# eth-ait/GaussianHaircut

Hardware: NVIDIA H100
Metric: fwd+bwd Gaussians/s at 500k G, 1080p (higher is better)
Workload: dtype f32

## Files before the change

### gaussianhaircut_b200/_C.py

```python
from __future__ import annotations

import ctypes as C
from typing import Optional, Tuple

import torch

from . import _capi
from ._alloc import empty_rows, row_capacity

NUM_CHANNELS = 10

_GRAD_LAYOUT = (("rotations", 4), ("colors", NUM_CHANNELS), ("opacity", 1), ("means3D", 3), ("scales", 3),
                ("means2D", 3), ("conic", 4), ("cov3D", 6))
_N_TRAINABLE_SEGMENTS = 5
GRAD_FLOATS_TRAINABLE_NATIVE = 4 + NUM_CHANNELS + 1 + 3 + 3
GRAD_FLOATS_PER_GAUSSIAN = sum(n for _, n in _GRAD_LAYOUT)


def _seg_floats(P: int, n: int) -> int:
    return (P * n + 3) // 4 * 4


def arena_floats(P: int) -> int:
    return sum(_seg_floats(P, n) for _, n in _GRAD_LAYOUT)


def trainable_floats(P: int) -> int:
    return sum(_seg_floats(P, n) for _, n in _GRAD_LAYOUT[:_N_TRAINABLE_SEGMENTS])


def _ptr(t: Optional[torch.Tensor]):
    if t is None or t.numel() == 0:
        return None
    return C.c_void_p(t.data_ptr())


def _prep(t: torch.Tensor, name: str, device: torch.device, align: int = 4) -> torch.Tensor:
    if t.numel() == 0:
        return t
    if t.dtype != torch.float32:
        raise RuntimeError(f"expected scalar type Float but found {t.dtype} for argument '{name}'")
    if t.device != device:
        raise RuntimeError(f"argument '{name}' is on {t.device}, expected {device}")
    t = t.contiguous()
    if t.data_ptr() % align:
        t = t.clone()
    return t


def _stream(device: torch.device):
    return C.c_void_p(torch.cuda.current_stream(device).cuda_stream)


def rasterize_gaussians(
    background: torch.Tensor, means3D: torch.Tensor, means2D_precomp: torch.Tensor,
    colors: torch.Tensor, opacity: torch.Tensor, scales: torch.Tensor, rotations: torch.Tensor,
    scale_modifier: float, cov3D_precomp: torch.Tensor, conic_precomp: torch.Tensor,
    viewmatrix: torch.Tensor, projmatrix: torch.Tensor, tan_fovx: float, tan_fovy: float,
    image_height: int, image_width: int, sh: torch.Tensor, degree: int, campos: torch.Tensor,
    prefiltered: bool, debug: bool,
) -> Tuple[int, torch.Tensor, torch.Tensor, torch.Tensor, torch.Tensor, torch.Tensor]:
    if means3D.ndim != 2 or means3D.size(1) != 3:
        raise RuntimeError("means3D must have dimensions (num_points, 3)")
    lib = _capi.load()
    device = means3D.device
    if device.type != "cuda":
        raise RuntimeError("gaussianhaircut_b200 rasterizer: tensors must live on a CUDA device (no CPU path)")
    P, H, W = int(means3D.size(0)), int(image_height), int(image_width)
    byte_opts = dict(dtype=torch.uint8, device=device)

    if P == 0:
        return (0, torch.zeros((NUM_CHANNELS, H, W), dtype=torch.float32, device=device),
                torch.zeros((0,), dtype=torch.int32, device=device),
                torch.empty(0, **byte_opts), torch.empty(0, **byte_opts), torch.empty(0, **byte_opts))

    with torch.cuda.device(device):
        means3D = _prep(means3D, "means3D", device)
        colors = _prep(colors, "colors", device, align=8)
        opacity = _prep(opacity, "opacity", device)
        scales = _prep(scales, "scales", device)
        rotations = _prep(rotations, "rotations", device, align=16)
        cov3D_precomp = _prep(cov3D_precomp, "cov3D_precomp", device)
        conic_precomp = _prep(conic_precomp, "conic_precomp", device)
        viewmatrix = _prep(viewmatrix, "viewmatrix", device)
        projmatrix = _prep(projmatrix, "projmatrix", device)
        background = _prep(background, "background", device)
        M = int(sh.size(1)) if sh.numel() != 0 else 0

        geom_bytes, img_bytes, geom_cap = C.c_size_t(), C.c_size_t(), C.c_size_t()
        _capi.check(lib.gh_forward_workspace_sizes(P, W, H, C.byref(geom_bytes), C.byref(img_bytes)))
        _capi.check(lib.gh_forward_workspace_sizes(row_capacity(P), W, H, C.byref(geom_cap), None))
        geomBuffer = torch.empty(geom_cap.value, **byte_opts)[:geom_bytes.value]
        imgBuffer = torch.empty(img_bytes.value, **byte_opts)
        radii = empty_rows(P, (), torch.int32, device)
        out_color = torch.empty((NUM_CHANNELS, H, W), dtype=torch.float32, device=device)
        stream = _stream(device)

        n_rendered, max_len = C.c_int(0), C.c_int(0)
        _capi.check(lib.gh_forward_preprocess(
            P, int(degree), M, W, H,
            _ptr(means3D), _ptr(means2D_precomp), _ptr(sh), _ptr(colors), _ptr(opacity),
            _ptr(scales), float(scale_modifier), _ptr(rotations),
            _ptr(cov3D_precomp), _ptr(conic_precomp),
            _ptr(viewmatrix), _ptr(projmatrix), _ptr(campos),
            float(tan_fovx), float(tan_fovy), int(bool(prefiltered)),
            _ptr(radii), _ptr(geomBuffer), _ptr(imgBuffer),
            C.byref(n_rendered), C.byref(max_len), int(bool(debug)), stream))
        R = int(n_rendered.value)

        bin_bytes = C.c_size_t()
        _capi.check(lib.gh_binning_workspace_size(R, C.byref(bin_bytes)))
        binningBuffer = torch.empty(bin_bytes.value, **byte_opts)
        _capi.check(lib.gh_forward_render(
            P, W, H, _ptr(background), _ptr(colors), _ptr(radii),
            _ptr(geomBuffer), _ptr(binningBuffer), _ptr(imgBuffer),
            R, int(max_len.value), _ptr(out_color), int(bool(debug)), stream))
    return R, out_color, radii, geomBuffer, binningBuffer, imgBuffer


def alloc_forward_workspaces(P: int, W: int, H: int, device: torch.device):
    lib = _capi.load()
    byte_opts = dict(dtype=torch.uint8, device=device)
    geom_bytes, img_bytes, geom_cap = C.c_size_t(), C.c_size_t(), C.c_size_t()
    _capi.check(lib.gh_forward_workspace_sizes(P, W, H, C.byref(geom_bytes), C.byref(img_bytes)))
    _capi.check(lib.gh_forward_workspace_sizes(row_capacity(P), W, H, C.byref(geom_cap), None))
    geomBuffer = torch.empty(geom_cap.value, **byte_opts)[:geom_bytes.value]
    imgBuffer = torch.empty(img_bytes.value, **byte_opts)
    radii = empty_rows(P, (), torch.int32, device)
    return geomBuffer, imgBuffer, radii


def forward_render(background: torch.Tensor, colors: torch.Tensor, radii: torch.Tensor, geomBuffer: torch.Tensor,
                   imgBuffer: torch.Tensor, num_rendered: int, max_tile_len: int, image_height: int, image_width: int,
                   debug: bool = False):
    lib = _capi.load()
    device = colors.device
    P, H, W = int(colors.shape[0]), int(image_height), int(image_width)
    with torch.cuda.device(device):
        background = _prep(background, "background", device)
        colors = _prep(colors, "colors", device, align=8)
        out_color = torch.empty((NUM_CHANNELS, H, W), dtype=torch.float32, device=device)
        bin_bytes = C.c_size_t()
        _capi.check(lib.gh_binning_workspace_size(int(num_rendered), C.byref(bin_bytes)))
        binningBuffer = torch.empty(bin_bytes.value, dtype=torch.uint8, device=device)
        _capi.check(lib.gh_forward_render(
            P, W, H, _ptr(background), _ptr(colors), _ptr(radii),
            _ptr(geomBuffer), _ptr(binningBuffer), _ptr(imgBuffer),
            int(num_rendered), int(max_tile_len), _ptr(out_color), int(bool(debug)), _stream(device)))
    return out_color, binningBuffer


def alloc_grad_arena(P: int, device: torch.device, zero: bool = True, storage: torch.Tensor | None = None):
    n = arena_floats(P)
    if storage is not None:
        if storage.dtype != torch.float32 or storage.numel() < n or not storage.is_contiguous():
            raise RuntimeError("gradient arena storage must be a contiguous float32 tensor of at least _C.arena_floats(P) elements")
        flat = storage.view(-1)[:n]
        if zero:
            flat.zero_()
    else:
        alloc = torch.zeros if zero else torch.empty
        flat = alloc(n, dtype=torch.float32, device=device)
    views, off = {}, 0
    for name, k in _GRAD_LAYOUT:
        views[name] = flat[off:off + P * k].view(P, k)
        off += _seg_floats(P, k)
    return flat, views


def rasterize_gaussians_backward_arena(
    background, means3D, radii, colors, scales, rotations, scale_modifier, cov3D_precomp, conic_precomp,
    viewmatrix, projmatrix, tan_fovx, tan_fovy, dL_dout_color, sh, degree, campos,
    geomBuffer, R, binningBuffer, imageBuffer, debug, arena_storage=None,
):
    lib = _capi.load()
    device = means3D.device
    P = int(means3D.size(0))
    H, W = int(dL_dout_color.size(1)), int(dL_dout_color.size(2))
    M = int(sh.size(1)) if sh.numel() != 0 else 0
    flat, g = alloc_grad_arena(P, device, zero=False, storage=arena_storage)
    dL_dsh = torch.zeros((P, M, 3), dtype=torch.float32, device=device)
    if P != 0:
        with torch.cuda.device(device):
            means3D = _prep(means3D, "means3D", device)
            colors = _prep(colors, "colors", device, align=8)
            scales = _prep(scales, "scales", device)
            rotations = _prep(rotations, "rotations", device, align=16)
            cov3D_precomp = _prep(cov3D_precomp, "cov3D_precomp", device)
            conic_precomp = _prep(conic_precomp, "conic_precomp", device)
            viewmatrix = _prep(viewmatrix, "viewmatrix", device)
            projmatrix = _prep(projmatrix, "projmatrix", device)
            background = _prep(background, "background", device)
            dL_dout_color = _prep(dL_dout_color, "dL_dout_color", device)
            radii = radii.contiguous()
            _capi.check(lib.gh_backward(
                P, int(degree), M, int(R), W, H,
                _ptr(background), _ptr(means3D), _ptr(sh), _ptr(colors),
                _ptr(scales), float(scale_modifier), _ptr(rotations),
                _ptr(cov3D_precomp), _ptr(conic_precomp),
                _ptr(viewmatrix), _ptr(projmatrix), _ptr(campos),
                float(tan_fovx), float(tan_fovy), _ptr(radii),
                _ptr(geomBuffer), _ptr(binningBuffer), _ptr(imageBuffer),
                _ptr(dL_dout_color),
                _ptr(g["means2D"]), _ptr(g["conic"]), _ptr(g["opacity"]), _ptr(g["colors"]),
                _ptr(g["means3D"]), _ptr(g["cov3D"]), _ptr(dL_dsh), _ptr(g["scales"]), _ptr(g["rotations"]),
                int(bool(debug)), _stream(device)))
    return flat, g, dL_dsh


def rasterize_gaussians_backward_records(background, means3D, radii, colors, conic_precomp, viewmatrix, projmatrix,
                                         tan_fovx, tan_fovy, dL_dout_color, campos, geomBuffer, R, binningBuffer,
                                         imageBuffer, debug) -> None:
    lib = _capi.load()
    device = means3D.device
    P = int(means3D.size(0))
    if P == 0:
        return
    H, W = int(dL_dout_color.size(1)), int(dL_dout_color.size(2))
    if conic_precomp is None or conic_precomp.numel() == 0:
        raise RuntimeError("rasterize_gaussians_backward_records needs the conic_precomp call shape")
    with torch.cuda.device(device):
        dL = _prep(dL_dout_color, "dL_dout_color", device)
        _capi.check(lib.gh_backward(
            P, 0, 0, int(R), W, H,
            _ptr(background), _ptr(means3D), None, _ptr(colors),
            None, 1.0, None, None, _ptr(conic_precomp),
            _ptr(viewmatrix), _ptr(projmatrix), _ptr(campos),
            float(tan_fovx), float(tan_fovy), _ptr(radii),
            _ptr(geomBuffer), _ptr(binningBuffer), _ptr(imageBuffer),
            _ptr(dL),
            None, None, None, None, None, None, None, None, None,
            int(bool(debug)), _stream(device)))


def rasterize_gaussians_backward(
    background: torch.Tensor, means3D: torch.Tensor, radii: torch.Tensor, colors: torch.Tensor,
    scales: torch.Tensor, rotations: torch.Tensor, scale_modifier: float,
    cov3D_precomp: torch.Tensor, conic_precomp: torch.Tensor,
    viewmatrix: torch.Tensor, projmatrix: torch.Tensor, tan_fovx: float, tan_fovy: float,
    dL_dout_color: torch.Tensor, sh: torch.Tensor, degree: int, campos: torch.Tensor,
    geomBuffer: torch.Tensor, R: int, binningBuffer: torch.Tensor, imageBuffer: torch.Tensor,
    debug: bool,
):
    _flat, g, dL_dsh = rasterize_gaussians_backward_arena(
        background, means3D, radii, colors, scales, rotations, scale_modifier, cov3D_precomp, conic_precomp,
        viewmatrix, projmatrix, tan_fovx, tan_fovy, dL_dout_color, sh, degree, campos,
        geomBuffer, R, binningBuffer, imageBuffer, debug)
    P = int(means3D.size(0))
    return (g["means2D"], g["colors"], g["opacity"], g["means3D"], g["cov3D"],
            g["conic"].view(P, 2, 2), dL_dsh, g["scales"], g["rotations"])


def mark_visible(means3D: torch.Tensor, viewmatrix: torch.Tensor, projmatrix: torch.Tensor) -> torch.Tensor:
    lib = _capi.load()
    device = means3D.device
    P = int(means3D.size(0))
    present = torch.zeros((P,), dtype=torch.bool, device=device)
    if P != 0:
        with torch.cuda.device(device):
            means3D = _prep(means3D, "means3D", device)
            viewmatrix = _prep(viewmatrix, "viewmatrix", device)
            projmatrix = _prep(projmatrix, "projmatrix", device)
            _capi.check(lib.gh_mark_visible(P, _ptr(means3D), _ptr(viewmatrix), _ptr(projmatrix),
                                            _ptr(present), _stream(device)))
    return present


def debug_export(P: int, W: int, H: int, R: int, geomBuffer, binningBuffer, imgBuffer):
    lib = _capi.load()
    device = geomBuffer.device
    T = ((W + 15) // 16) * ((H + 15) // 16)
    out = {
        "keys": torch.zeros(R, dtype=torch.int64, device=device),
        "point_list": torch.zeros(R, dtype=torch.int32, device=device),
        "ranges": torch.zeros((T, 2), dtype=torch.int32, device=device),
        "final_T": torch.zeros(H * W, dtype=torch.float32, device=device),
        "n_contrib": torch.zeros(H * W, dtype=torch.int32, device=device),
        "depths": torch.zeros(P, dtype=torch.float32, device=device),
        "means2D": torch.zeros((P, 2), dtype=torch.float32, device=device),
        "conic_opacity": torch.zeros((P, 4), dtype=torch.float32, device=device),
    }
    with torch.cuda.device(device):
        _capi.check(lib.gh_debug_export(
            P, W, H, R, _ptr(geomBuffer), _ptr(binningBuffer), _ptr(imgBuffer),
            _ptr(out["keys"]), _ptr(out["point_list"]), _ptr(out["ranges"]),
            _ptr(out["final_T"]), _ptr(out["n_contrib"]),
            _ptr(out["depths"]), _ptr(out["means2D"]), _ptr(out["conic_opacity"]), _stream(device)))
    return out
```

### gaussianhaircut_b200/_capi.py

```python
from __future__ import annotations

import ctypes as C
import os

_HERE = os.path.dirname(os.path.abspath(__file__))
LIB_PATH = os.path.join(_HERE, "lib", "libgh_raster.so")

GH_OK = 0
GH_E_INVALID_ARG = 1
GH_E_NO_COLORS = 2
GH_E_CUDA = 3
GH_E_PREFILTERED = 4

ABI_VERSION = 3

_p = C.c_void_p
_i = C.c_int
_f = C.c_float
_ll = C.c_longlong
_sz = C.c_size_t

SIGNATURES = {
    "gh_abi_version": (_i, []),
    "gh_num_channels": (_i, []),
    "gh_last_error": (C.c_char_p, []),
    "gh_kernel_launch_count": (C.c_ulonglong, []),
    "gh_stage_timing_enable": (None, [_i]),
    "gh_stage_timing_read": (_i, [C.POINTER(C.c_double), C.POINTER(C.c_ulonglong), _i]),
    "gh_forward_workspace_sizes": (_i, [_i, _i, _i, C.POINTER(_sz), C.POINTER(_sz)]),
    "gh_binning_workspace_size": (_i, [_ll, C.POINTER(_sz)]),
    "gh_forward_preprocess": (_i, [
        _i, _i, _i, _i, _i,
        _p, _p, _p, _p, _p,
        _p, _f, _p,
        _p, _p,
        _p, _p, _p,
        _f, _f, _i,
        _p,
        _p, _p,
        C.POINTER(_i), C.POINTER(_i),
        _i, _p]),
    "gh_forward_render": (_i, [
        _i, _i, _i, _p, _p, _p, _p, _p, _p, _i, _i, _p, _i, _p]),
    "gh_backward": (_i, [
        _i, _i, _i, _i, _i, _i,
        _p,
        _p, _p, _p,
        _p, _f, _p,
        _p, _p,
        _p, _p, _p,
        _f, _f,
        _p,
        _p, _p, _p,
        _p,
        _p, _p, _p, _p,
        _p, _p, _p, _p, _p,
        _i, _p]),
    "gh_mark_visible": (_i, [_i, _p, _p, _p, _p, _p]),
    "gh_adam_step": (_i, [_i, _p, _p, _p, _p, _p, _p, _f, _f, _f, _i, _p, _p, _p, _p]),
    "gh_image_loss_workspace_size": (_i, [_i, _i, C.POINTER(C.c_size_t)]),
    "gh_allreduce_p2p": (_i, [_p, _p, C.c_ulonglong, _i, _i, C.c_size_t, C.c_size_t, C.c_uint, _p, _p, _p]),
    "gh_image_loss": (_i, [_i, _i, _p, _p, _p, _p, _p, _f, _f, _f, _f, _p, _p, _p, _p]),
    "gh_project_workspace_size": (_i, [_i, C.POINTER(C.c_size_t)]),
    "gh_project_forward": (_i, [
        _i, _i, _i,
        _p, _p, _p, _p,
        _p, _p,
        _p, _p, _p,
        _p, _p, _p,
        _f, _f, _f, _i, C.c_uint, _f,
        _p, _p, _p, _p, _p, _p,
        _p]),
    "gh_project_forward_binned": (_i, [
        _i, _i, _i,
        _p, _p, _p, _p,
        _p, _p,
        _p, _p, _p,
        _p, _p, _p,
        _f, _f, _f, _i, C.c_uint, _f,
        _p, _p, _p, _p, _p, _p,
        _p, _p, _p, C.POINTER(C.c_int), C.POINTER(C.c_int),
        _p]),
    "gh_project_backward": (_i, [
        _i, _i, _i,
        _p, _p, _p, _p,
        _p, _p,
        _p, _p, _p,
        _p, _p, _p,
        _f, _f, _f, _i, C.c_uint, _f,
        _p,
        _p,
        _p, _p, _p, _p,
        _p, _p, _p, _p, _p, _p,
        _p, _p, _p, _p, _p,
        _p, _p, _p]),
    "gh_densify_classify": (_i, [_i, _p, _p, _p, _p, _f, _f, _f, _f, _p, _p]),
    "gh_densify_scatter": (_i, [_i, _i, _p, _p, _p, _p, _p, _p, _p, _i, _i, _i, _p, _p, _i, _i, _i, _p, _i, _p]),
    "gh_debug_export": (_i, [_i, _i, _i, _ll, _p, _p, _p, _p, _p, _p, _p, _p, _p, _p, _p, _p]),
}

_lib = None


class GhError(RuntimeError):

    def __init__(self, code: int, message: str):
        super().__init__(message)
        self.code = code


def load() -> C.CDLL:
    global _lib
    if _lib is not None:
        return _lib
    if not os.path.isfile(LIB_PATH):
        raise RuntimeError(
            f"gaussianhaircut_b200: native library not found at {LIB_PATH}. "
            "Build it with `python -m gaussianhaircut_b200.build` (needs nvcc; there is no CPU fallback).")
    lib = C.CDLL(LIB_PATH)
    for name, (res, args) in SIGNATURES.items():
        fn = getattr(lib, name)
        fn.restype = res
        fn.argtypes = args
    if lib.gh_abi_version() != ABI_VERSION:
        raise RuntimeError(f"libgh_raster.so ABI {lib.gh_abi_version()} != binding ABI {ABI_VERSION}; rebuild")
    _lib = lib
    return lib


STAGE_NAMES = ("preprocess", "tile_scan", "emit", "tile_sort", "blend_forward", "blend_backward",
               "preprocess_backward")


def stage_timing_read():
    lib = load()
    n = len(STAGE_NAMES)
    ms = (C.c_double * n)()
    calls = (C.c_ulonglong * n)()
    lib.gh_stage_timing_read(ms, calls, n)
    return {STAGE_NAMES[i]: (ms[i], int(calls[i])) for i in range(n)}


def check(status: int) -> None:
    if status != GH_OK:
        msg = load().gh_last_error().decode("utf-8", "replace")
        raise GhError(status, msg or f"libgh_raster error {status}")
```

### gaussianhaircut_b200/csrc/gh_api.cu

```cuda
#include "gh_common.cuh"
#include "gh_kernels.h"
#include "../../include/gh_rasterizer.h"

#include <atomic>
#include <cstdio>
#include <cstring>
#include <mutex>

static thread_local char g_err[512] = "";
void gh_clear_error() { g_err[0] = 0; }
int gh_set_error(int code, const char* msg) {
    std::snprintf(g_err, sizeof(g_err), "%s", msg ? msg : "");
    return code;
}

namespace {

int gh_fail(int code, const char* msg) { return gh_set_error(code, msg); }

int gh_check_cuda(cudaError_t e, const char* what) {
    if (e == cudaSuccess) return GH_OK;
    std::snprintf(g_err, sizeof(g_err), "[CUDA ERROR] %s: %s", what, cudaGetErrorString(e));
    return GH_E_CUDA;
}

#define GH_STAGE(stream, debug, what)                                             \
    do {                                                                           \
        cudaError_t e__ = cudaGetLastError();                                      \
        if (e__ == cudaSuccess && (debug)) e__ = cudaStreamSynchronize(stream);    \
        if (e__ != cudaSuccess) return gh_check_cuda(e__, what);                   \
    } while (0)

enum { GH_ST_PREPROCESS = 0, GH_ST_TILE_SCAN, GH_ST_EMIT, GH_ST_TILE_SORT, GH_ST_BLEND_FWD, GH_ST_BLEND_BWD,
       GH_ST_PREPROCESS_BWD, GH_ST_COUNT };
std::atomic<bool> g_timing{false};
std::mutex g_timing_mu;
double g_stage_ms[GH_ST_COUNT] = {0};
unsigned long long g_stage_calls[GH_ST_COUNT] = {0};
std::atomic<unsigned long long> g_launches{0};

struct GhStageTimer {
    int stage; cudaStream_t stream; unsigned long long l0; bool on;
    cudaEvent_t ev0 = nullptr, ev1 = nullptr;
    GhStageTimer(int st, cudaStream_t s) : stage(st), stream(s), l0(g_launches.load()), on(g_timing.load()) {
        if (on) {
            on = (cudaEventCreate(&ev0) == cudaSuccess) && (cudaEventCreate(&ev1) == cudaSuccess);
            if (on) cudaEventRecord(ev0, stream);
        }
    }
    ~GhStageTimer() {
        if (on && g_launches.load() != l0) {
            cudaEventRecord(ev1, stream);
            cudaEventSynchronize(ev1);
            float ms = 0.f;
            if (cudaEventElapsedTime(&ms, ev0, ev1) == cudaSuccess) {
                std::lock_guard<std::mutex> lk(g_timing_mu);
                g_stage_ms[stage] += ms; g_stage_calls[stage] += 1;
            }
        }
        if (ev0) cudaEventDestroy(ev0);
        if (ev1) cudaEventDestroy(ev1);
    }
};

inline void gh_grid(int W, int H, int& gx, int& gy) {
    gx = (W + GH_BLOCK_X - 1) / GH_BLOCK_X;
    gy = (H + GH_BLOCK_Y - 1) / GH_BLOCK_Y;
}

__global__ void gh_export_keys_kernel(const uint2* __restrict__ ranges, const uint64_t* __restrict__ inst,
                                      unsigned long long* __restrict__ keys, unsigned int* __restrict__ plist)
{
    const uint2 rg = ranges[blockIdx.x];
    for (uint32_t i = rg.x + threadIdx.x; i < rg.y; i += blockDim.x) {
        const uint64_t r = inst[i];
        if (keys) keys[i] = ((unsigned long long)blockIdx.x << 32) | (r >> 32);
        if (plist) plist[i] = (unsigned int)r;
    }
}

__global__ void gh_export_geom_kernel(int P, const GhGeo* __restrict__ geo, float* __restrict__ means2D,
                                      float* __restrict__ conic_opacity)
{
    const int i = blockIdx.x * blockDim.x + threadIdx.x;
    if (i >= P) return;
    const GhGeo g = geo[i];
    if (means2D) { means2D[2 * i] = g.x; means2D[2 * i + 1] = g.y; }
    if (conic_opacity) {
        conic_opacity[4 * i + 0] = g.ca; conic_opacity[4 * i + 1] = g.cb;
        conic_opacity[4 * i + 2] = g.cc; conic_opacity[4 * i + 3] = g.op;
    }
}

}

void gh_count_launches(int n) { g_launches.fetch_add((unsigned long long)n); }

extern "C" {

int gh_abi_version(void) { return 3; }

unsigned long long gh_kernel_launch_count(void) { return g_launches.load(); }

void gh_stage_timing_enable(int on) {
    std::lock_guard<std::mutex> lk(g_timing_mu);
    g_timing.store(on != 0);
    for (int i = 0; i < GH_ST_COUNT; i++) { g_stage_ms[i] = 0.0; g_stage_calls[i] = 0; }
}

int gh_stage_timing_read(double* ms_sum, unsigned long long* calls, int capacity) {
    std::lock_guard<std::mutex> lk(g_timing_mu);
    const int n = capacity < GH_ST_COUNT ? capacity : GH_ST_COUNT;
    for (int i = 0; i < n; i++) { if (ms_sum) ms_sum[i] = g_stage_ms[i]; if (calls) calls[i] = g_stage_calls[i]; }
    return GH_ST_COUNT;
}
int gh_num_channels(void) { return GH_NUM_CHANNELS; }
const char* gh_last_error(void) { return g_err; }

int gh_forward_workspace_sizes(int P, int width, int height, size_t* geom_bytes, size_t* img_bytes)
{
    if (P < 0 || width <= 0 || height <= 0) return gh_fail(GH_E_INVALID_ARG, "gh_forward_workspace_sizes: bad P/width/height");
    int gx, gy; gh_grid(width, height, gx, gy);
    if (geom_bytes) *geom_bytes = GhGeomWS::bytes((size_t)P);
    if (img_bytes) *img_bytes = GhImgWS::bytes((size_t)width * height, (size_t)gx * gy);
    return GH_OK;
}

int gh_binning_workspace_size(long long R, size_t* binning_bytes)
{
    if (R < 0) return gh_fail(GH_E_INVALID_ARG, "gh_binning_workspace_size: negative R");
    if (binning_bytes) *binning_bytes = GhBinWS::bytes((size_t)R);
    return GH_OK;
}

int gh_forward_preprocess(
    int P, int D, int M, int width, int height,
    const float* means3D, const float* means2D_precomp, const float* shs,
    const float* colors_precomp, const float* opacities,
    const float* scales, float scale_modifier, const float* rotations,
    const float* cov3D_precomp, const float* conic_precomp,
    const float* viewmatrix, const float* projmatrix, const float* cam_pos,
    float tan_fovx, float tan_fovy, int prefiltered,
    int* radii, char* geom_buffer, char* img_buffer,
    int* num_rendered, int* max_tile_len, int debug, gh_stream_t stream_)
{
    (void)D; (void)M; (void)means2D_precomp; (void)shs; (void)cam_pos;
    cudaStream_t stream = (cudaStream_t)stream_;
    g_err[0] = 0;
    if (P <= 0 || width <= 0 || height <= 0) return gh_fail(GH_E_INVALID_ARG, "gh_forward_preprocess: P, width, height must be positive");
    if (colors_precomp == nullptr)
        return gh_fail(GH_E_NO_COLORS, "For non-RGB, provide precomputed Gaussian colors!");
    if (!means3D || !opacities || !viewmatrix || !projmatrix || !radii || !geom_buffer || !img_buffer || !num_rendered)
        return gh_fail(GH_E_INVALID_ARG, "gh_forward_preprocess: missing mandatory pointer");
    if (conic_precomp == nullptr && cov3D_precomp == nullptr && (scales == nullptr || rotations == nullptr))
        return gh_fail(GH_E_INVALID_ARG, "Please provide exactly one of either scale/rotation pair or precomputed 3D covariance!");
    if (rotations && ((size_t)rotations & 15)) return gh_fail(GH_E_INVALID_ARG, "rotations must be 16-byte aligned");
    if (((size_t)colors_precomp & 7)) return gh_fail(GH_E_INVALID_ARG, "colors_precomp must be 8-byte aligned");

    int gx, gy; gh_grid(width, height, gx, gy);
    const int T = gx * gy;
    if ((unsigned long long)gx * gx * gy >= (1ull << 32))
        return gh_fail(GH_E_INVALID_ARG, "gh_forward_preprocess: image too large (tile grid gx * gx * gy must stay below 2^32)");
    GhGeomWS geom = GhGeomWS::carve(geom_buffer, (size_t)P);
    GhImgWS img = GhImgWS::carve(img_buffer, (size_t)width * height, (size_t)T);

    cudaError_t e = cudaMemsetAsync(img.ctrl, 0, 256 + gh_align_up((size_t)T * 4, 256), stream);
    if (e != cudaSuccess) return gh_check_cuda(e, "memset(tile histogram)");

    {
        GhStageTimer t(GH_ST_PREPROCESS, stream);
        gh_launch_preprocess(P, means3D, scales, scale_modifier, rotations, opacities, cov3D_precomp,
                             conic_precomp, viewmatrix, projmatrix, width, height, tan_fovx, tan_fovy,
                             radii, geom, img, prefiltered, stream);
        g_launches += 1;
    }
    GH_STAGE(stream, debug, "preprocess");
    {
        GhStageTimer t(GH_ST_TILE_SCAN, stream);
        gh_launch_tile_scan(T, img, stream);
        g_launches += 1;
    }
    GH_STAGE(stream, debug, "tile scan");
    GhCtrl h;
    e = cudaMemcpyAsync(&h, img.ctrl, sizeof(GhCtrl), cudaMemcpyDeviceToHost, stream);
    if (e == cudaSuccess) e = cudaStreamSynchronize(stream);
    if (e != cudaSuccess) return gh_check_cuda(e, "read back num_rendered");
    *num_rendered = (int)h.num_rendered;
    if (max_tile_len) *max_tile_len = (int)h.max_tile_len;
    if (h.err_flags & GH_ERR_PREFILTERED)
        return gh_fail(GH_E_PREFILTERED, "Point is filtered although prefiltered is set. This shouldn't happen!");
    return GH_OK;
}

int gh_forward_render(
    int P, int width, int height,
    const float* background, const float* colors_precomp, const int* radii,
    char* geom_buffer, char* binning_buffer, char* img_buffer,
    int num_rendered, int max_tile_len, float* out_color, int debug, gh_stream_t stream_)
{
    cudaStream_t stream = (cudaStream_t)stream_;
    g_err[0] = 0;
    if (P <= 0 || width <= 0 || height <= 0 || num_rendered < 0) return gh_fail(GH_E_INVALID_ARG, "gh_forward_render: bad sizes");
    if (!background || !colors_precomp || !radii || !geom_buffer || !img_buffer || !out_color || (num_rendered > 0 && !binning_buffer))
        return gh_fail(GH_E_INVALID_ARG, "gh_forward_render: missing mandatory pointer");
    int gx, gy; gh_grid(width, height, gx, gy);
    const int T = gx * gy;
    GhGeomWS geom = GhGeomWS::carve(geom_buffer, (size_t)P);
    GhImgWS img = GhImgWS::carve(img_buffer, (size_t)width * height, (size_t)T);
    GhBinWS bin = GhBinWS::carve(binning_buffer, (size_t)num_rendered);

    if (num_rendered > 0) {
        {
            GhStageTimer t(GH_ST_EMIT, stream);
            gh_launch_emit(P, radii, geom, img, bin, gx, gy, stream);
            g_launches += 1;
        }
        GH_STAGE(stream, debug, "emit");
        {
            GhStageTimer t(GH_ST_TILE_SORT, stream);
            g_launches += gh_launch_tile_sort(T, (unsigned int)max_tile_len, (long long)num_rendered, img, bin, stream);
        }
        GH_STAGE(stream, debug, "tile sort");
    }
    {
        GhStageTimer t(GH_ST_BLEND_FWD, stream);
        gh_launch_blend_forward(width, height, gx, gy, geom, img, bin, colors_precomp, background, out_color, stream);
        g_launches += 1;
    }
    GH_STAGE(stream, debug, "blend forward");
    return GH_OK;
}

int gh_backward(
    int P, int D, int M, int R, int width, int height,
    const float* background,
    const float* means3D, const float* shs, const float* colors_precomp,
    const float* scales, float scale_modifier, const float* rotations,
    const float* cov3D_precomp, const float* conic_precomp,
    const float* viewmatrix, const float* projmatrix, const float* campos,
    float tan_fovx, float tan_fovy, const int* radii,
    char* geom_buffer, char* binning_buffer, char* img_buffer,
    const float* dL_dpix,
    float* dL_dmean2D, float* dL_dconic, float* dL_dopacity, float* dL_dcolor,
    float* dL_dmean3D, float* dL_dcov3D, float* dL_dsh, float* dL_dscale, float* dL_drot,
    int debug, gh_stream_t stream_)
{
    (void)D; (void)M; (void)shs; (void)campos; (void)dL_dsh;
    cudaStream_t stream = (cudaStream_t)stream_;
    g_err[0] = 0;
    if (P <= 0 || width <= 0 || height <= 0 || R < 0) return gh_fail(GH_E_INVALID_ARG, "gh_backward: bad sizes");
    const bool keep_records = (conic_precomp != nullptr) && !dL_dmean2D && !dL_dconic && !dL_dopacity && !dL_dcolor;
    if (!background || !means3D || !colors_precomp || !viewmatrix || !projmatrix || !radii ||
        !geom_buffer || !img_buffer || !dL_dpix || (R > 0 && !binning_buffer) ||
        (!keep_records && (!dL_dmean2D || !dL_dconic || !dL_dopacity || !dL_dcolor)))
        return gh_fail(GH_E_INVALID_ARG, "gh_backward: missing mandatory pointer");
    if (conic_precomp == nullptr) {
        if (!dL_dmean3D || !dL_dcov3D) return gh_fail(GH_E_INVALID_ARG, "gh_backward: dL_dmean3D/dL_dcov3D required");
        if (cov3D_precomp == nullptr && (!scales || !rotations || !dL_dscale || !dL_drot))
            return gh_fail(GH_E_INVALID_ARG, "gh_backward: scales/rotations and their gradient buffers required");
        if (rotations && ((size_t)rotations & 15)) return gh_fail(GH_E_INVALID_ARG, "rotations must be 16-byte aligned");
        if (dL_drot && ((size_t)dL_drot & 15)) return gh_fail(GH_E_INVALID_ARG, "dL_drot must be 16-byte aligned");
    }
    if (((size_t)colors_precomp & 7)) return gh_fail(GH_E_INVALID_ARG, "colors_precomp must be 8-byte aligned");
    if (((size_t)dL_dconic & 15)) return gh_fail(GH_E_INVALID_ARG, "dL_dconic must be 16-byte aligned");
    if (((size_t)dL_dcolor & 7)) return gh_fail(GH_E_INVALID_ARG, "dL_dcolor must be 8-byte aligned");
    if (keep_records && (dL_dmean3D || dL_dcov3D || dL_dscale || dL_drot))
        return gh_fail(GH_E_INVALID_ARG, "gh_backward: geometry gradients cannot be requested without the 2-D gradient outputs");
    int gx, gy; gh_grid(width, height, gx, gy);
    const int T = gx * gy;
    GhGeomWS geom = GhGeomWS::carve(geom_buffer, (size_t)P);
    GhImgWS img = GhImgWS::carve(img_buffer, (size_t)width * height, (size_t)T);
    GhBinWS bin = GhBinWS::carve(binning_buffer, (size_t)R);

    if (R == 0 && keep_records) {
        cudaError_t e = cudaMemsetAsync(geom.acc16, 0, (size_t)P * 64, stream);
        if (e != cudaSuccess) return gh_check_cuda(e, "memset(accumulation records)");
    }
    if (R == 0) {
        struct { float* p; size_t n; } z[] = {{dL_dmean2D, 3}, {dL_dconic, 4}, {dL_dopacity, 1}, {dL_dcolor, GH_NUM_CHANNELS},
                                              {dL_dmean3D, 3}, {dL_dcov3D, 6}, {dL_dscale, 3}, {dL_drot, 4}};
        for (auto& b : z)
            if (b.p) {
                cudaError_t e = cudaMemsetAsync(b.p, 0, (size_t)P * b.n * sizeof(float), stream);
                if (e != cudaSuccess) return gh_check_cuda(e, "memset(gradients)");
            }
    }
    if (R > 0) {
        GhStageTimer t(GH_ST_BLEND_BWD, stream);
        cudaError_t e = cudaMemsetAsync(geom.acc16, 0, (size_t)P * 64, stream);
        if (e != cudaSuccess) return gh_check_cuda(e, "memset(accumulation records)");
        gh_launch_blend_backward(width, height, gx, gy, geom, img, bin, colors_precomp, background, dL_dpix, stream);
        g_launches += 1;
        if (conic_precomp != nullptr && !keep_records) {
            gh_launch_unpack_grads(P, geom, dL_dmean2D, dL_dconic, dL_dopacity, dL_dcolor,
                                   dL_dmean3D, dL_dcov3D, dL_dscale, dL_drot, stream);
            g_launches += 1;
        }
    }
    GH_STAGE(stream, debug, "blend backward");
    if (conic_precomp == nullptr && R > 0) {
        GhStageTimer t(GH_ST_PREPROCESS_BWD, stream);
        gh_launch_preprocess_backward(P, means3D, radii, scales, scale_modifier, rotations, cov3D_precomp,
                                      conic_precomp, viewmatrix, projmatrix, width, height, tan_fovx, tan_fovy,
                                      geom.acc16, dL_dmean2D, dL_dconic, dL_dopacity, dL_dcolor,
                                      dL_dmean3D, dL_dcov3D, dL_dscale, dL_drot, stream);
        g_launches += 1;
    }
    GH_STAGE(stream, debug, "preprocess backward");
    return GH_OK;
}

int gh_mark_visible(int P, const float* means3D, const float* viewmatrix, const float* projmatrix,
                    unsigned char* present, gh_stream_t stream_)
{
    (void)projmatrix;
    cudaStream_t stream = (cudaStream_t)stream_;
    g_err[0] = 0;
    if (P < 0) return gh_fail(GH_E_INVALID_ARG, "gh_mark_visible: negative P");
    if (P == 0) return GH_OK;
    if (!means3D || !viewmatrix || !present) return gh_fail(GH_E_INVALID_ARG, "gh_mark_visible: missing pointer");
    gh_launch_mark_visible(P, means3D, viewmatrix, reinterpret_cast<bool*>(present), stream);
    GH_STAGE(stream, 0, "mark visible");
    return GH_OK;
}

int gh_debug_export(
    int P, int width, int height, long long R,
    const char* geom_buffer, const char* binning_buffer, const char* img_buffer,
    unsigned long long* keys_sorted, unsigned int* point_list, unsigned int* ranges,
    float* final_T, unsigned int* n_contrib,
    float* depths, float* means2D, float* conic_opacity, gh_stream_t stream_)
{
    cudaStream_t stream = (cudaStream_t)stream_;
    g_err[0] = 0;
    if (P <= 0 || width <= 0 || height <= 0 || R < 0 || !geom_buffer || !img_buffer)
        return gh_fail(GH_E_INVALID_ARG, "gh_debug_export: bad arguments");
    int gx, gy; gh_grid(width, height, gx, gy);
    const int T = gx * gy;
    const size_t npix = (size_t)width * height;
    GhGeomWS geom = GhGeomWS::carve(const_cast<char*>(geom_buffer), (size_t)P);
    GhImgWS img = GhImgWS::carve(const_cast<char*>(img_buffer), npix, (size_t)T);
    cudaError_t e = cudaSuccess;
    if (R > 0 && binning_buffer && (keys_sorted || point_list)) {
        GhBinWS bin = GhBinWS::carve(const_cast<char*>(binning_buffer), (size_t)R);
        gh_export_keys_kernel<<<T, 128, 0, stream>>>(img.ranges, bin.inst, keys_sorted, point_list);
    }
    if (ranges && e == cudaSuccess) e = cudaMemcpyAsync(ranges, img.ranges, (size_t)T * 8, cudaMemcpyDeviceToDevice, stream);
    if (final_T && e == cudaSuccess) e = cudaMemcpyAsync(final_T, img.final_T, npix * 4, cudaMemcpyDeviceToDevice, stream);
    if (n_contrib && e == cudaSuccess) e = cudaMemcpyAsync(n_contrib, img.n_contrib, npix * 4, cudaMemcpyDeviceToDevice, stream);
    if (depths && e == cudaSuccess) e = cudaMemcpyAsync(depths, geom.depth, (size_t)P * 4, cudaMemcpyDeviceToDevice, stream);
    if ((means2D || conic_opacity) && e == cudaSuccess)
        gh_export_geom_kernel<<<(P + 255) / 256, 256, 0, stream>>>(P, geom.geo, means2D, conic_opacity);
    if (e != cudaSuccess) return gh_check_cuda(e, "debug export");
    GH_STAGE(stream, 0, "debug export");
    return GH_OK;
}

}
```

### gaussianhaircut_b200/csrc/gh_blend.cu

```cuda
#include "gh_common.cuh"
#include "gh_kernels.h"

#define GH_HALF_C (GH_NUM_CHANNELS / 2)

#ifndef GH_TILE_ORDER
#define GH_TILE_ORDER 1
#endif
#ifndef GH_FWD_NBUF
#define GH_FWD_NBUF 1
#endif
#ifndef GH_FWD_CHUNK
#define GH_FWD_CHUNK 384
#endif
#ifndef GH_FWD_MIN_CTAS
#define GH_FWD_MIN_CTAS 6
#endif
#ifndef GH_FWD_SMEM_MIN
#define GH_FWD_SMEM_MIN 0
#endif
#ifndef GH_BWD_CHUNK
#define GH_BWD_CHUNK 384
#endif
#ifndef GH_BWD_MIN_CTAS
#define GH_BWD_MIN_CTAS 6
#endif
#ifndef GH_BWD_LPB
#define GH_BWD_LPB 2
#endif
#define GH_BWD_NBLK (128 / GH_BWD_LPB)
#define GH_BWD_BPW (32 / GH_BWD_LPB)
#define GH_BWD_BW GH_BWD_LPB
#define GH_BWD_NBX (16 / GH_BWD_BW)
#ifndef GH_ABLATE_REDG
#define GH_ABLATE_REDG 0
#endif
#ifndef GH_BWD_FAST_EXP
#define GH_BWD_FAST_EXP 0
#endif

namespace {

struct GhPixEval {
    float dx, dy, power, G, alpha;
    bool ok;
};

__device__ __forceinline__ GhPixEval gh_eval(const float4 g0, const float4 g1, float pxf, float pyf) {
    GhPixEval e;
    e.dx = GH_SUB(g0.x, pxf);
    e.dy = GH_SUB(g0.y, pyf);
    e.power = gh_power(e.dx, e.dy, g0.z, g0.w, g1.x);
    e.G = 0.f; e.alpha = 0.f;
    e.ok = false;
    if (!(e.power > 0.0f)) {
        e.G = expf(e.power);
        e.alpha = fminf(0.99f, GH_MUL(g1.y, e.G));
        e.ok = !(e.alpha < 1.0f / 255.0f);
    }
    return e;
}

__device__ __forceinline__ void gh_cp_async16(void* smem, const void* gmem) {
    const unsigned s = (unsigned)__cvta_generic_to_shared(smem);
    asm volatile("cp.async.cg.shared.global [%0], [%1], 16;\n" ::"r"(s), "l"(gmem));
}
__device__ __forceinline__ void gh_cp_async8(void* smem, const void* gmem) {
    const unsigned s = (unsigned)__cvta_generic_to_shared(smem);
    asm volatile("cp.async.ca.shared.global [%0], [%1], 8;\n" ::"r"(s), "l"(gmem));
}
__device__ __forceinline__ void gh_cp_async_commit() { asm volatile("cp.async.commit_group;\n" ::); }
__device__ __forceinline__ void gh_cp_async_wait_all() { asm volatile("cp.async.wait_group 0;\n" ::: "memory"); }

__device__ __forceinline__ float2 gh_f2(float a) { return make_float2(a, a); }
__device__ __forceinline__ float2 gh_neg2(float2 a) { return make_float2(-a.x, -a.y); }
__device__ __forceinline__ float2 gh_mul2(float2 a, float2 b) { return make_float2(__fmul_rn(a.x, b.x), __fmul_rn(a.y, b.y)); }
__device__ __forceinline__ float2 gh_add2(float2 a, float2 b) { return make_float2(__fadd_rn(a.x, b.x), __fadd_rn(a.y, b.y)); }
__device__ __forceinline__ float2 gh_sub2(float2 a, float2 b) { return gh_add2(a, gh_neg2(b)); }
__device__ __forceinline__ float2 gh_fma2(float2 a, float2 b, float2 c) { return make_float2(__fmaf_rn(a.x, b.x, c.x), __fmaf_rn(a.y, b.y, c.y)); }
__device__ __forceinline__ float gh_rcp_approx(float x) {
    float r;
    asm("rcp.approx.ftz.f32 %0, %1;" : "=f"(r) : "f"(x));
    return r;
}

#define GH_FWD_THREADS 128
#define GH_FWD_WORDS (GH_FWD_CHUNK / 32)
static_assert(GH_FWD_CHUNK % 32 == 0 && GH_FWD_WORDS <= 32, "forward window: a multiple of 32 records, at most 1024");

struct GhStage {
    float4 g0[GH_FWD_NBUF][GH_FWD_CHUNK];
    float4 g1[GH_FWD_NBUF][GH_FWD_CHUNK];
    float2 feat[GH_FWD_NBUF][GH_FWD_CHUNK * GH_HALF_C];
};
constexpr size_t kFwdStageBytes = sizeof(GhStage) + (size_t)GH_FWD_WORDS * GH_FWD_THREADS * sizeof(uint32_t);
constexpr size_t kFwdSortBytes = 16u * GH_INKERNEL_SORT_MAX + 4u * GH_SORT_SCRATCH_WORDS;
constexpr size_t kFwdSmemBytes = kFwdStageBytes > kFwdSortBytes ? kFwdStageBytes : kFwdSortBytes;

__device__ __forceinline__ void gh_stage_issue(GhStage& st, int buf, int slot, uint32_t id,
                                               const GhGeo* __restrict__ geo, const float* __restrict__ features) {
    const float4* gp = reinterpret_cast<const float4*>(geo + id);
    gh_cp_async16(&st.g0[buf][slot], gp);
    gh_cp_async16(&st.g1[buf][slot], gp + 1);
    const float2* fp = reinterpret_cast<const float2*>(features + (size_t)id * GH_NUM_CHANNELS);
#pragma unroll
    for (int k = 0; k < GH_HALF_C; k++) gh_cp_async8(&st.feat[buf][slot * GH_HALF_C + k], fp + k);
}

__device__ __forceinline__ uint32_t gh_transpose32(uint32_t x, int lane) {
#pragma unroll
    for (int s = 16; s >= 1; s >>= 1) {
        const uint32_t m = (s == 16) ? 0x0000ffffu : (s == 8) ? 0x00ff00ffu : (s == 4) ? 0x0f0f0f0fu
                         : (s == 2) ? 0x33333333u : 0x55555555u;
        const uint32_t y = __shfl_xor_sync(0xffffffffu, x, s);
        x = (lane & s) ? (((y >> s) & m) | (x & ~m)) : ((x & m) | ((y & m) << s));
    }
    return x;
}

__device__ __forceinline__ void gh_build_pair_lists(const GhStage& st, uint32_t* pairbits, int buf, int cnt,
                                                    int word, int lane, float tx0, float ty0) {
    const int j = word * 32 + lane;
    uint32_t pairmask[8];
#pragma unroll
    for (int t = 0; t < 8; t++) pairmask[t] = 0u;
    float gx = 0.f, gy = 0.f, b = 0.f, ia = 0.f, aQ = -1.f, bbac = 0.f;
    int r0 = 16, r1 = -1;
    bool all_pixels = false;
    if (j < cnt) {
        const float4 g0 = st.g0[buf][j], g1 = st.g1[buf][j];
        gx = g0.x; gy = g0.y; b = g0.w;
        const float a = g0.z, c = g1.x, thr = g1.z, pd = g1.w;
        const float mxd = fmaxf(fabsf(gx - tx0), fabsf(gx - (tx0 + 15.f)));
        const float myd = fmaxf(fabsf(gy - ty0), fabsf(gy - (ty0 + 15.f)));
        const float slack = 1e-3f + 2e-5f * (a * mxd * mxd + c * myd * myd + 2.f * fabsf(b) * mxd * myd);
        const float Q = 2.f * (thr + slack);
        if (pd == 0.f || Q != Q) {
            all_pixels = true; r0 = 0; r1 = 15;
        } else if (Q >= 0.f) {
            ia = __frcp_rn(a);
            aQ = a * Q;
            bbac = b * b - a * c;
            const float ry = sqrtf(aQ / (-bbac)) + 0.01f;
            r0 = 0; r1 = 15;
            if (ry == ry) { r0 = max(0, __float2int_ru(gy - ry - ty0)); r1 = min(15, __float2int_rd(gy + ry - ty0)); }
        }
    }
    int wr0 = r0, wr1 = r1;
#pragma unroll
    for (int o = 16; o > 0; o >>= 1) {
        wr0 = min(wr0, __shfl_xor_sync(0xffffffffu, wr0, o));
        wr1 = max(wr1, __shfl_xor_sync(0xffffffffu, wr1, o));
    }
    const float2 bbac2 = gh_f2(bbac), aQ2 = gh_f2(aQ), b2 = gh_f2(b), ia2 = gh_f2(ia), gx2 = gh_f2(gx);
    const float2 off2 = gh_f2(-0.01f), ntx2 = gh_f2(-tx0);
#pragma unroll
    for (int t = 0; t < 8; t++) {
        if (2 * t + 1 < wr0 || 2 * t > wr1) continue;
        const float2 dy = make_float2(gy - (ty0 + (float)(2 * t)), gy - (ty0 + (float)(2 * t + 1)));
        const float2 disc = gh_fma2(gh_mul2(dy, dy), bbac2, aQ2);
        const float2 sq = gh_mul2(disc, make_float2(rsqrtf(disc.x), rsqrtf(disc.y)));
        const float2 hb = gh_mul2(b2, dy);
        const float2 lo = gh_add2(gh_add2(gh_fma2(gh_sub2(hb, sq), ia2, gx2), off2), ntx2);
        const float2 hi = gh_add2(gh_add2(gh_fma2(gh_add2(hb, sq), ia2, gx2), gh_neg2(off2)), ntx2);
        const int p0a = max(0, __float2int_ru(lo.x)), p1a = min(15, __float2int_rd(hi.x));
        const int p0b = max(0, __float2int_ru(lo.y)), p1b = min(15, __float2int_rd(hi.y));
        const uint32_t ma = (disc.x > 0.f && p0a <= p1a) ? (((2u << (p1a - p0a)) - 1u) << p0a) : 0u;
        const uint32_t mb = (disc.y > 0.f && p0b <= p1b) ? (((2u << (p1b - p0b)) - 1u) << p0b) : 0u;
        pairmask[t] = all_pixels ? 0xffffu : (ma | mb);
    }
#pragma unroll
    for (int w = 0; w < GH_FWD_THREADS / 32; w++) {
        const uint32_t m = pairmask[2 * w] | (pairmask[2 * w + 1] << 16);
        uint32_t col = 0u;
        if (__any_sync(0xffffffffu, m != 0u)) col = gh_transpose32(m, lane);
        pairbits[word * GH_FWD_THREADS + w * 32 + lane] = col;
    }
}

__global__ void __launch_bounds__(GH_FWD_THREADS, GH_FWD_MIN_CTAS)
gh_blend_forward_kernel(const uint2* __restrict__ ranges, const uint32_t* __restrict__ tile_perm, uint64_t* inst,
                        const GhGeo* __restrict__ geo, const float* __restrict__ features,
                        int W, int H, int gx, const float* __restrict__ bg,
                        float* __restrict__ final_T, uint32_t* __restrict__ n_contrib,
                        float* __restrict__ out)
{
    extern __shared__ __align__(16) unsigned char gh_fwd_smem[];
    GhStage& st = *reinterpret_cast<GhStage*>(gh_fwd_smem);
    uint32_t* pairbits = reinterpret_cast<uint32_t*>(gh_fwd_smem + sizeof(GhStage));

    const int tile = GH_TILE_ORDER ? (int)tile_perm[blockIdx.x] : (int)blockIdx.x;
    const int tx = tile % gx, ty = tile / gx;
    const int tid = threadIdx.x, lane = tid & 31, warp = tid >> 5;
    const int px = tx * GH_BLOCK_X + (lane & 15);
    const int py0 = ty * GH_BLOCK_Y + 4 * warp + 2 * (lane >> 4);
    const bool inside0 = (px < W) && (py0 < H), inside1 = (px < W) && (py0 + 1 < H);
    const float pxf = (float)px, pyf0 = (float)py0, pyf1 = (float)(py0 + 1);
    const float tx0 = (float)(tx * GH_BLOCK_X), ty0 = (float)(ty * GH_BLOCK_Y);

    const uint2 rg = ranges[tile];
    const int n = (int)(rg.y - rg.x);
    const int nchunks = (n + GH_FWD_CHUNK - 1) / GH_FWD_CHUNK;

    float2 T = make_float2(1.0f, 1.0f);
    float2 C[GH_NUM_CHANNELS];
#pragma unroll
    for (int ch = 0; ch < GH_NUM_CHANNELS; ch++) C[ch] = make_float2(0.f, 0.f);
    uint32_t last0 = 0, last1 = 0;
    bool done0 = !inside0, done1 = !inside1;
    bool warp_done = (__ballot_sync(0xffffffffu, done0 && done1) == 0xffffffffu);

#ifndef GH_ABLATE_SORT
#define GH_ABLATE_SORT 0
#endif
#ifndef GH_ABLATE_TRAVERSE
#define GH_ABLATE_TRAVERSE 0
#endif
#ifndef GH_ABLATE_BUILD
#define GH_ABLATE_BUILD 0
#endif
#ifndef GH_ABLATE_GATHER
#define GH_ABLATE_GATHER 0
#endif
    if (!GH_ABLATE_SORT && n >= 2 && n <= (int)GH_INKERNEL_SORT_MAX) {
        uint64_t* sbase = reinterpret_cast<uint64_t*>(gh_fwd_smem);
        uint64_t* spong = sbase + GH_INKERNEL_SORT_MAX;
        uint32_t* sscratch = reinterpret_cast<uint32_t*>(spong + GH_INKERNEL_SORT_MAX);
        uint64_t* gl = inst + rg.x;
        const uint32_t odd = rg.x & 1u;
        const uint32_t nrec = ((uint32_t)n + odd + 1u) & ~1u;
        uint64_t* skeys = sbase;
        if (nrec <= GH_INKERNEL_SORT_MAX) {
            skeys = sbase + odd;
            __shared__ __align__(8) uint64_t s_mbar;
            const uint32_t mbar = (uint32_t)__cvta_generic_to_shared(&s_mbar);
            if (tid == 0) {
                asm volatile("mbarrier.init.shared::cta.b64 [%0], 1;" ::"r"(mbar) : "memory");
                asm volatile("fence.mbarrier_init.release.cluster;" ::: "memory");
            }
            __syncthreads();
            if (tid == 0) {
                const uint32_t bytes = nrec * 8u;
                asm volatile("mbarrier.arrive.expect_tx.shared::cta.b64 _, [%0], %1;" ::"r"(mbar), "r"(bytes) : "memory");
                asm volatile("cp.async.bulk.shared::cluster.global.mbarrier::complete_tx::bytes [%0], [%1], %2, [%3];"
                             ::"r"((uint32_t)__cvta_generic_to_shared(sbase)), "l"(gl - odd), "r"(bytes), "r"(mbar) : "memory");
            }
            uint32_t landed = 0;
            for (uint32_t it = 0; it < (1u << 24) && !landed; it++)
                asm volatile("{\n .reg .pred p;\n mbarrier.try_wait.parity.shared::cta.b64 p, [%1], 0;\n selp.u32 %0, 1, 0, p;\n}"
                             : "=r"(landed) : "r"(mbar) : "memory");
            if (!landed) __trap();
        } else {
            for (int i = tid; i < n; i += GH_FWD_THREADS) skeys[i] = gl[i];
            __syncthreads();
        }
        if (n <= 64) gh_bitonic_sort(skeys, (uint32_t)n, tid, GH_FWD_THREADS);
        else gh_bucket_sort_tile<GH_FWD_THREADS>(skeys, spong, sscratch, n, tid);
        for (int i = tid; i < n; i += GH_FWD_THREADS) gl[i] = skeys[i];
        __syncthreads();
    }

    constexpr int PER_THREAD = (GH_FWD_CHUNK + GH_FWD_THREADS - 1) / GH_FWD_THREADS;
    uint32_t next_id[PER_THREAD];
#pragma unroll
    for (int h = 0; h < PER_THREAD; h++) {
        const int slot = tid + h * GH_FWD_THREADS;
        next_id[h] = (slot < GH_FWD_CHUNK && slot < n) ? (uint32_t)inst[(size_t)rg.x + slot] : 0u;
    }
    auto stage_window = [&](int c, int buf) {
        const int wbase = c * GH_FWD_CHUNK;
#pragma unroll
        for (int h = 0; h < PER_THREAD; h++) {
            const int slot = tid + h * GH_FWD_THREADS;
            if (!GH_ABLATE_GATHER && slot < GH_FWD_CHUNK && wbase + slot < n) gh_stage_issue(st, buf, slot, next_id[h], geo, features);
        }
        gh_cp_async_commit();
#pragma unroll
        for (int h = 0; h < PER_THREAD; h++) {
            const int slot = tid + h * GH_FWD_THREADS, nx = wbase + GH_FWD_CHUNK + slot;
            if (slot < GH_FWD_CHUNK && nx < n) next_id[h] = (uint32_t)inst[(size_t)rg.x + nx];
        }
    };
#if GH_FWD_NBUF == 2
    if (nchunks > 0) stage_window(0, 0);
#endif

    for (int c = 0; c < nchunks; c++) {
        const int base = c * GH_FWD_CHUNK;
        const int cnt = min(GH_FWD_CHUNK, n - base);
        const int nwords = (cnt + 31) >> 5;
#if GH_FWD_NBUF == 2
        const int buf = c & 1;
        gh_cp_async_wait_all();
        if (__syncthreads_and(warp_done)) break;
        if (c + 1 < nchunks) stage_window(c + 1, buf ^ 1);
#else
        constexpr int buf = 0;
        if (__syncthreads_and(warp_done)) break;
        stage_window(c, 0);
        gh_cp_async_wait_all();
        __syncthreads();
#endif
        if (!GH_ABLATE_BUILD)
            for (int word = warp; word < nwords; word += GH_FWD_THREADS / 32)
                gh_build_pair_lists(st, pairbits, buf, cnt, word, lane, tx0, ty0);
        __syncthreads();

        if (!(done0 && done1) && !GH_ABLATE_TRAVERSE) {
            uint32_t nz = 0u;
#pragma unroll
            for (int k = 0; k < GH_FWD_WORDS; k++)
                if (k < nwords) nz |= (pairbits[k * GH_FWD_THREADS + tid] != 0u) ? (1u << k) : 0u;
            int wi = 0;
            uint32_t cur = 0u;
            while (true) {
                if (cur == 0u) {
                    if (nz == 0u) break;
                    wi = __ffs(nz) - 1;
                    nz &= nz - 1;
                    cur = pairbits[wi * GH_FWD_THREADS + tid];
                }
                const int bpos = __ffs(cur) - 1;
                cur &= cur - 1;
                const int jj = wi * 32 + bpos;
                const float4 g0 = st.g0[buf][jj], g1 = st.g1[buf][jj];
                const GhPixEval e0 = gh_eval(g0, g1, pxf, pyf0), e1 = gh_eval(g0, g1, pxf, pyf1);
                const float2 test_T = make_float2(GH_MUL(T.x, GH_SUB(1.0f, e0.alpha)), GH_MUL(T.y, GH_SUB(1.0f, e1.alpha)));
                const bool ok0 = !done0 && e0.ok, ok1 = !done1 && e1.ok;
                const bool stop0 = ok0 && test_T.x < 0.0001f, stop1 = ok1 && test_T.y < 0.0001f;
                const bool blend0 = ok0 && !stop0, blend1 = ok1 && !stop1;
                done0 = done0 || stop0;
                done1 = done1 || stop1;
                if (blend0 || blend1) {
                    const uint32_t pos = (uint32_t)(base + jj + 1);
#pragma unroll
                    for (int k = 0; k < GH_HALF_C; k++) {
                        const float2 f = st.feat[buf][jj * GH_HALF_C + k];
#pragma unroll
                        for (int h = 0; h < 2; h++) {
                            const float fc = h ? f.y : f.x;
                            float2& Cc = C[2 * k + h];
                            const float c0 = GH_FMA(T.x, GH_MUL(e0.alpha, fc), Cc.x);
                            const float c1 = GH_FMA(T.y, GH_MUL(e1.alpha, fc), Cc.y);
                            Cc = make_float2(blend0 ? c0 : Cc.x, blend1 ? c1 : Cc.y);
                        }
                    }
                    T = make_float2(blend0 ? test_T.x : T.x, blend1 ? test_T.y : T.y);
                    last0 = blend0 ? pos : last0;
                    last1 = blend1 ? pos : last1;
                }
                if (done0 && done1) break;
            }
        }
        warp_done = (__ballot_sync(0xffffffffu, done0 && done1) == 0xffffffffu);
    }
    gh_cp_async_wait_all();

    const size_t plane = (size_t)H * W;
#pragma unroll
    for (int r = 0; r < 2; r++) {
        if (!(r ? inside1 : inside0)) continue;
        const size_t pix = (size_t)(py0 + r) * W + px;
        const float Tr = r ? T.y : T.x;
        final_T[pix] = Tr;
        n_contrib[pix] = r ? last1 : last0;
#pragma unroll
        for (int ch = 0; ch < GH_NUM_CHANNELS; ch++)
            out[ch * plane + pix] = GH_FMA(Tr, __ldg(bg + ch), r ? C[ch].y : C[ch].x);
    }
}

struct GhStageB {
    float4 g0[GH_BWD_CHUNK];
    float4 g1[GH_BWD_CHUNK];
    float2 feat[GH_BWD_CHUNK * GH_HALF_C];
    uint32_t id[GH_BWD_CHUNK];
    uint32_t bits[GH_BWD_NBLK][GH_BWD_CHUNK / 32 + 1];
};

__device__ __forceinline__ void gh_stage_issue_b(GhStageB& st, int slot, uint32_t id,
                                                 const GhGeo* __restrict__ geo, const float* __restrict__ features) {
    const float4* gp = reinterpret_cast<const float4*>(geo + id);
    gh_cp_async16(&st.g0[slot], gp);
    gh_cp_async16(&st.g1[slot], gp + 1);
    const float2* fp = reinterpret_cast<const float2*>(features + (size_t)id * GH_NUM_CHANNELS);
#pragma unroll
    for (int k = 0; k < GH_HALF_C; k++) gh_cp_async8(&st.feat[slot * GH_HALF_C + k], fp + k);
    st.id[slot] = id;
}

#if GH_BWD_LPB == 4
__device__ __forceinline__ uint32_t gh_block_mask2(const float4 g0, const float4 g1, float tx0, float ty0) {
    const float gx = g0.x, gy = g0.y, a = g0.z, b = g0.w, c = g1.x, thr = g1.z, pd = g1.w;
    if (pd == 0.f) return 0xffffffffu;
    const float mxd = fmaxf(fabsf(gx - tx0), fabsf(gx - (tx0 + 15.f)));
    const float myd = fmaxf(fabsf(gy - ty0), fabsf(gy - (ty0 + 15.f)));
    const float slack = 1e-3f + 2e-5f * (a * mxd * mxd + c * myd * myd + 2.f * fabsf(b) * mxd * myd);
    const float Q = 2.f * (thr + slack);
    if (!(Q >= 0.f)) return (Q != Q) ? 0xffffffffu : 0u;
    const float2 ia = gh_f2(__frcp_rn(a)), aQ = gh_f2(a * Q), bbac = gh_f2(b * b - a * c), gx2 = gh_f2(gx), b2 = gh_f2(b);
    float2 dy = make_float2(gy - ty0, gy - (ty0 + 1.f));
    uint32_t mask = 0;
#pragma unroll
    for (int by = 0; by < 8; by++) {
        const float2 disc = gh_fma2(gh_mul2(dy, dy), bbac, aQ);
        const float2 s = gh_mul2(disc, make_float2(rsqrtf(disc.x), rsqrtf(disc.y)));
        const float2 hb = gh_mul2(b2, dy);
        const float2 lo2 = gh_fma2(gh_sub2(hb, s), ia, gx2), hi2 = gh_fma2(gh_add2(hb, s), ia, gx2);
        const float xlo = fminf(fminf(1e30f, lo2.x), lo2.y), xhi = fmaxf(fmaxf(-1e30f, hi2.x), hi2.y);
        const float lo = (xlo - 0.01f) - tx0, hi = (xhi + 0.01f) - tx0;
        const int p0 = max(0, __float2int_ru(lo)), p1 = min(15, __float2int_rd(hi));
        if (p0 <= p1) {
            const int b0 = p0 >> 2, b1 = p1 >> 2;
            mask |= (((2u << (b1 - b0)) - 1u) << b0) << (4 * by);
        }
        dy = gh_add2(dy, gh_f2(-2.f));
    }
    return mask;
}
#endif

#if GH_BWD_LPB != 4
__device__ __forceinline__ uint2 gh_block_mask_2x2(const float4 g0, const float4 g1, float tx0, float ty0) {
    const float gx = g0.x, gy = g0.y, a = g0.z, b = g0.w, c = g1.x, thr = g1.z, pd = g1.w;
    if (pd == 0.f) return make_uint2(0xffffffffu, 0xffffffffu);
    const float mxd = fmaxf(fabsf(gx - tx0), fabsf(gx - (tx0 + 15.f)));
    const float myd = fmaxf(fabsf(gy - ty0), fabsf(gy - (ty0 + 15.f)));
    const float slack = 1e-3f + 2e-5f * (a * mxd * mxd + c * myd * myd + 2.f * fabsf(b) * mxd * myd);
    const float Q = 2.f * (thr + slack);
    if (!(Q >= 0.f)) return (Q != Q) ? make_uint2(0xffffffffu, 0xffffffffu) : make_uint2(0u, 0u);
    const float2 ia = gh_f2(__frcp_rn(a)), aQ = gh_f2(a * Q), bbac = gh_f2(b * b - a * c), gx2 = gh_f2(gx), b2 = gh_f2(b);
    float2 dy = make_float2(gy - ty0, gy - (ty0 + 1.f));
    uint32_t m[2] = {0u, 0u};
#pragma unroll 1
    for (int half = 0; half < 2; half++) {
        uint32_t mh = 0u;
#pragma unroll
        for (int by = 0; by < 4; by++) {
            const float2 disc = gh_fma2(gh_mul2(dy, dy), bbac, aQ);
            const float2 s = gh_mul2(disc, make_float2(rsqrtf(disc.x), rsqrtf(disc.y)));
            const float2 hb = gh_mul2(b2, dy);
            const float2 lo2 = gh_fma2(gh_sub2(hb, s), ia, gx2), hi2 = gh_fma2(gh_add2(hb, s), ia, gx2);
            const float xlo = fminf(fminf(1e30f, lo2.x), lo2.y), xhi = fmaxf(fmaxf(-1e30f, hi2.x), hi2.y);
            const float lo = (xlo - 0.01f) - tx0, hi = (xhi + 0.01f) - tx0;
            const int p0 = max(0, __float2int_ru(lo)), p1 = min(15, __float2int_rd(hi));
            if (p0 <= p1) {
                const int b0 = p0 >> 1, b1 = p1 >> 1;
                mh |= (((2u << (b1 - b0)) - 1u) << b0) << (8 * by);
            }
            dy = gh_add2(dy, gh_f2(-2.f));
        }
        if (half == 0) m[0] = mh; else m[1] = mh;
    }
    return make_uint2(m[0], m[1]);
}
#endif

__device__ __forceinline__ uint32_t gh_valid_bits(uint32_t glast, int first_pos) {
    const int lim = (int)glast - first_pos;
    return lim >= 32 ? 0xffffffffu : (lim <= 0 ? 0u : ((1u << lim) - 1u));
}

__device__ __forceinline__ void gh_build_lists_b(GhStageB& st, int cnt, int word, int lane, float tx0, float ty0,
                                                 int base, uint32_t glast_lo, uint32_t glast_hi) {
    const int j = word * 32 + lane;
#if GH_BWD_LPB == 4
    uint32_t m = 0;
    if (j < cnt) m = gh_block_mask2(st.g0[j], st.g1[j], tx0, ty0);
    uint32_t mine = 0;
    if (__any_sync(0xffffffffu, m != 0u)) mine = gh_transpose32(m, lane);
    st.bits[lane][word] = mine & gh_valid_bits(glast_lo, base + word * 32);
    (void)glast_hi;
#else
    uint2 m = make_uint2(0u, 0u);
    if (j < cnt) m = gh_block_mask_2x2(st.g0[j], st.g1[j], tx0, ty0);
    uint32_t lo = 0, hi = 0;
    if (__any_sync(0xffffffffu, m.x != 0u)) lo = gh_transpose32(m.x, lane);
    if (__any_sync(0xffffffffu, m.y != 0u)) hi = gh_transpose32(m.y, lane);
    st.bits[lane][word] = lo & gh_valid_bits(glast_lo, base + word * 32);
    st.bits[32 + lane][word] = hi & gh_valid_bits(glast_hi, base + word * 32);
#endif
}

#define GH_BWD_THREADS 128

#define GH_RED_STRIDE4 5
#if GH_BWD_LPB == 4
__device__ __forceinline__ float4 gh_group4_reduce16(const float (&v)[16], float4* warp_buf, int lane) {
    float4* mine = warp_buf + lane * GH_RED_STRIDE4;
    mine[0] = make_float4(v[0], v[1], v[2], v[3]);
    mine[1] = make_float4(v[4], v[5], v[6], v[7]);
    mine[2] = make_float4(v[8], v[9], v[10], v[11]);
    mine[3] = make_float4(v[12], v[13], v[14], v[15]);
    __syncwarp();
    const float4* grp = warp_buf + (lane & 28) * GH_RED_STRIDE4 + (lane & 3);
    const float4 a = grp[0], b = grp[GH_RED_STRIDE4], c = grp[2 * GH_RED_STRIDE4], d = grp[3 * GH_RED_STRIDE4];
    __syncwarp();
    const float2 lo = gh_add2(gh_add2(make_float2(a.x, a.y), make_float2(b.x, b.y)),
                              gh_add2(make_float2(c.x, c.y), make_float2(d.x, d.y)));
    const float2 hi = gh_add2(gh_add2(make_float2(a.z, a.w), make_float2(b.z, b.w)),
                              gh_add2(make_float2(c.z, c.w), make_float2(d.z, d.w)));
    return make_float4(lo.x, lo.y, hi.x, hi.y);
}
#endif

#ifndef GH_BWD_RED2_SECTOR
#define GH_BWD_RED2_SECTOR 1
#endif
#if GH_BWD_LPB != 4
__device__ __forceinline__ void gh_group2_reduce16(const float (&v)[16], int lane, float4& out0, float4& out1) {
    const bool odd = (lane & 1) != 0;
    constexpr int H = GH_BWD_RED2_SECTOR ? 4 : 8;
    float k[8];
#pragma unroll
    for (int i = 0; i < 8; i++) {
        const int c = GH_BWD_RED2_SECTOR ? ((i & 3) + 8 * (i >> 2)) : i;
        const float send = odd ? v[c] : v[c + H], keep = odd ? v[c + H] : v[c];
        k[i] = keep + __shfl_xor_sync(0xffffffffu, send, 1);
    }
    out0 = make_float4(k[0], k[1], k[2], k[3]);
    out1 = make_float4(k[4], k[5], k[6], k[7]);
}
#endif
#if GH_BWD_LPB == 4
#define GH_RED_LANE_STRIDE4 GH_RED_STRIDE4
#else
#define GH_RED_LANE_STRIDE4 0
#endif

struct GhBwdPair {
    float2 T, A, last_alpha, last_cdot;
    float2 ntf_bg;
    float2 npy;
    uint32_t last0, last1;
    float2 dL0[GH_HALF_C], dL1[GH_HALF_C];
};

__device__ __forceinline__ bool gh_bwd_pair(GhBwdPair& p, const float4 g0, const float4 g1, const float2* feat,
                                            float pxf, uint32_t pos, float nddelx_dx, float nddely_dy, float (&v)[16]) {
    const float dx = GH_SUB(g0.x, pxf);
    const float2 dx2 = gh_f2(dx);
    const float2 dy = gh_add2(gh_f2(g0.y), p.npy);
    const float t1 = GH_MUL(dx, g0.z), dxcb = GH_MUL(dx, g0.w);
    const float2 t3 = gh_mul2(dy, gh_mul2(dy, gh_f2(g1.x)));
    const float2 sq = gh_fma2(dx2, gh_f2(t1), t3);
    const float2 power = gh_fma2(sq, gh_f2(-0.5f), gh_mul2(dy, gh_f2(-dxcb)));
#if GH_BWD_FAST_EXP
    const float Gx0 = __expf((power.x > 0.0f) ? 0.0f : power.x);
    const float Gx1 = __expf((power.y > 0.0f) ? 0.0f : power.y);
#else
    const float Gx0 = expf((power.x > 0.0f) ? 0.0f : power.x);
    const float Gx1 = expf((power.y > 0.0f) ? 0.0f : power.y);
#endif
    const float2 ao = gh_mul2(gh_f2(g1.y), make_float2(Gx0, Gx1));
    const float alpha0 = fminf(0.99f, ao.x), alpha1 = fminf(0.99f, ao.y);
    const bool ok0 = (pos < p.last0) & !(power.x > 0.0f) & !(alpha0 < 1.0f / 255.0f);
    const bool ok1 = (pos < p.last1) & !(power.y > 0.0f) & !(alpha1 < 1.0f / 255.0f);
    const float2 am = make_float2(ok0 ? alpha0 : 0.f, ok1 ? alpha1 : 0.f);
    const float2 G = make_float2(ok0 ? Gx0 : 0.f, ok1 ? Gx1 : 0.f);
    const float2 om = gh_sub2(gh_f2(1.0f), am);
    const float2 r = make_float2(gh_rcp_approx(om.x), gh_rcp_approx(om.y));
    p.T = gh_mul2(p.T, r);
    const float2 w = gh_mul2(am, p.T);
    const float2 w0 = gh_f2(w.x), w1 = gh_f2(w.y);
    float2 c0, c1;
#pragma unroll
    for (int k = 0; k < GH_HALF_C; k++) {
        const float2 f = feat[k];
        c0 = (k == 0) ? gh_mul2(f, p.dL0[0]) : gh_fma2(f, p.dL0[k], c0);
        c1 = (k == 0) ? gh_mul2(f, p.dL1[0]) : gh_fma2(f, p.dL1[k], c1);
        const float2 vc = gh_fma2(w1, p.dL1[k], gh_mul2(w0, p.dL0[k]));
        v[2 * k] = vc.x; v[2 * k + 1] = vc.y;
    }
    const float2 cdot = make_float2(c0.x + c0.y, c1.x + c1.y);
    const float2 A_new = gh_fma2(p.last_alpha, gh_sub2(p.last_cdot, p.A), p.A);
    const float2 dL_dalpha = gh_fma2(gh_sub2(cdot, A_new), p.T, gh_mul2(p.ntf_bg, r));
    p.A = A_new;
    p.last_cdot = cdot;
    p.last_alpha = am;
    const float2 q = gh_mul2(G, dL_dalpha), qdy = gh_mul2(q, dy);
    const float S0 = q.x + q.y, S1 = qdy.x + qdy.y, S2 = fmaf(qdy.y, dy.y, qdy.x * dy.x);
    const float U0 = g1.y * S0, U1 = g1.y * S1;
    const float hdx = -0.5f * dx;
    v[10] = fmaf(t1, U0, g0.w * U1) * nddelx_dx;
    v[11] = fmaf(g1.x, U1, dxcb * U0) * nddely_dy;
    v[12] = (hdx * dx) * U0;
    v[13] = hdx * U1;
    v[14] = (-0.5f * g1.y) * S2;
    v[15] = S0;
    return ok0 | ok1;
}

__global__ void __launch_bounds__(GH_BWD_THREADS, GH_BWD_MIN_CTAS)
gh_blend_backward_kernel(const uint2* __restrict__ ranges, const uint32_t* __restrict__ tile_perm, const uint64_t* __restrict__ inst,
                         const GhGeo* __restrict__ geo, const float* __restrict__ features,
                         int W, int H, int gx, const float* __restrict__ bg,
                         const float* __restrict__ final_T, const uint32_t* __restrict__ n_contrib,
                         const float* __restrict__ dL_dpix,
                         float* __restrict__ acc16)
{
    extern __shared__ __align__(16) unsigned char gh_bwd_smem[];
    GhStageB& st = *reinterpret_cast<GhStageB*>(gh_bwd_smem);
#if GH_BWD_LPB == 4
    float4* red_buf = reinterpret_cast<float4*>(gh_bwd_smem + sizeof(GhStageB)) + (threadIdx.x >> 5) * 32 * GH_RED_LANE_STRIDE4;
#endif
    __shared__ uint32_t s_warp_last[GH_BWD_THREADS / 32];
    __shared__ uint32_t s_glast[GH_BWD_NBLK];
    __shared__ uint8_t s_perm[GH_BWD_THREADS / 32][GH_BWD_NBLK];

    const int tile = GH_TILE_ORDER ? (int)tile_perm[blockIdx.x] : (int)blockIdx.x;
    const int tx = tile % gx, ty = tile / gx;
    const int tid = threadIdx.x, lane = tid & 31, warp = tid >> 5;
    const float tx0 = (float)(tx * GH_BLOCK_X), ty0 = (float)(ty * GH_BLOCK_Y);
    const unsigned gshift = lane & (32 - GH_BWD_LPB);
    const unsigned gmask = (1u << GH_BWD_LPB) - 1u;
    const size_t plane = (size_t)H * W;
    const uint2 rg = ranges[tile];

    {
        const int nb = GH_BWD_BPW * warp + lane / GH_BWD_LPB;
        const int nx = tx * GH_BLOCK_X + GH_BWD_BW * (nb % GH_BWD_NBX) + (lane % GH_BWD_LPB);
        const int ny = ty * GH_BLOCK_Y + 2 * (nb / GH_BWD_NBX);
        uint32_t gl = 0;
        if (nx < W && ny < H) gl = n_contrib[(size_t)ny * W + nx];
        if (nx < W && ny + 1 < H) gl = max(gl, n_contrib[(size_t)(ny + 1) * W + nx]);
#pragma unroll
        for (int o = GH_BWD_LPB / 2; o > 0; o >>= 1) gl = max(gl, __shfl_xor_sync(0xffffffffu, gl, o));
        if ((lane % GH_BWD_LPB) == 0) s_glast[nb] = gl;
        uint32_t wl = gl;
#pragma unroll
        for (int o = GH_BWD_LPB; o < 32; o <<= 1) wl = max(wl, __shfl_xor_sync(0xffffffffu, wl, o));
        if (lane == 0) s_warp_last[warp] = wl;
    }
    __syncthreads();
    uint32_t tile_last = 0;
#pragma unroll
    for (int w = 0; w < GH_BWD_THREADS / 32; w++) tile_last = max(tile_last, s_warp_last[w]);
    const int n = (int)tile_last;
    const int nchunks = (n + GH_BWD_CHUNK - 1) / GH_BWD_CHUNK;
    if (nchunks == 0) return;
    constexpr int PER_THREAD = (GH_BWD_CHUNK + GH_BWD_THREADS - 1) / GH_BWD_THREADS;
#define GH_GLAST_LO s_glast[lane]
#define GH_GLAST_HI ((GH_BWD_NBLK > 32) ? s_glast[(32 + lane) % GH_BWD_NBLK] : 0u)

    uint32_t next_id[PER_THREAD];
    {
        const int base = (nchunks - 1) * GH_BWD_CHUNK;
        const int cnt = n - base;
#pragma unroll
        for (int h = 0; h < PER_THREAD; h++) {
            const int slot = tid + h * GH_BWD_THREADS;
            if (slot < cnt) gh_stage_issue_b(st, slot, (uint32_t)inst[(size_t)rg.x + base + slot], geo, features);
        }
        gh_cp_async_commit();
        if (nchunks > 1) {
#pragma unroll
            for (int h = 0; h < PER_THREAD; h++)
                if (tid + h * GH_BWD_THREADS < GH_BWD_CHUNK)
                    next_id[h] = (uint32_t)inst[(size_t)rg.x + base - GH_BWD_CHUNK + tid + h * GH_BWD_THREADS];
        }
        gh_cp_async_wait_all();
        __syncthreads();
        for (int word = warp; word * 32 < cnt; word += GH_BWD_THREADS / 32)
            gh_build_lists_b(st, cnt, word, lane, tx0, ty0, base, GH_GLAST_LO, GH_GLAST_HI);
        __syncthreads();
    }

    int blk;
    {
        const int nw = (n - (nchunks - 1) * GH_BWD_CHUNK + 31) >> 5;
        uint32_t len0 = 0, len1 = 0;
        for (int w = 0; w < nw; w++) {
            len0 += __popc(st.bits[lane][w]);
            if (GH_BWD_NBLK > 32) len1 += __popc(st.bits[(32 + lane) % GH_BWD_NBLK][w]);
        }
        const uint32_t key0 = (len0 << 6) | (uint32_t)lane, key1 = (len1 << 6) | (uint32_t)(32 + lane);
        int rank0 = 0, rank1 = 0;
#pragma unroll
        for (int k = 0; k < 32; k++) {
            const uint32_t a = __shfl_sync(0xffffffffu, key0, k);
            rank0 += (a < key0) ? 1 : 0;
            if (GH_BWD_NBLK > 32) {
                const uint32_t b = __shfl_sync(0xffffffffu, key1, k);
                rank0 += (b < key0) ? 1 : 0;
                rank1 += ((a < key1) ? 1 : 0) + ((b < key1) ? 1 : 0);
            }
        }
        s_perm[warp][rank0] = (uint8_t)lane;
        if (GH_BWD_NBLK > 32) s_perm[warp][rank1] = (uint8_t)(32 + lane);
        __syncwarp();
        blk = s_perm[warp][GH_BWD_BPW * warp + lane / GH_BWD_LPB];
    }
    const int px = tx * GH_BLOCK_X + GH_BWD_BW * (blk % GH_BWD_NBX) + (lane % GH_BWD_LPB);
    const int py0 = ty * GH_BLOCK_Y + 2 * (blk / GH_BWD_NBX);
    const float pxf = (float)px;

    GhBwdPair pr;
    {
        float tf[2], bgd[2];
        uint32_t lastv[2];
#pragma unroll
        for (int r = 0; r < 2; r++) {
            const int py = py0 + r;
            const bool inside = (px < W) && (py < H);
            const size_t pi = (size_t)py * W + px;
            tf[r] = inside ? final_T[pi] : 0.f;
            lastv[r] = inside ? n_contrib[pi] : 0u;
            float d[GH_NUM_CHANNELS];
            bgd[r] = 0.f;
#pragma unroll
            for (int ch = 0; ch < GH_NUM_CHANNELS; ch++) {
                d[ch] = inside ? dL_dpix[ch * plane + pi] : 0.f;
                bgd[r] += __ldg(bg + ch) * d[ch];
            }
#pragma unroll
            for (int k = 0; k < GH_HALF_C; k++) {
                if (r == 0) pr.dL0[k] = make_float2(d[2 * k], d[2 * k + 1]);
                else pr.dL1[k] = make_float2(d[2 * k], d[2 * k + 1]);
            }
        }
        pr.T = make_float2(tf[0], tf[1]);
        pr.ntf_bg = make_float2(-tf[0] * bgd[0], -tf[1] * bgd[1]);
        pr.npy = make_float2(-(float)py0, -(float)(py0 + 1));
        pr.A = gh_f2(0.f); pr.last_alpha = gh_f2(0.f); pr.last_cdot = gh_f2(0.f);
        pr.last0 = lastv[0]; pr.last1 = lastv[1];
    }
    const float nddelx_dx = -0.5f * W, nddely_dy = -0.5f * H;

    uint32_t wlast = s_glast[blk];
#pragma unroll
    for (int o = GH_BWD_LPB; o < 32; o <<= 1) wlast = max(wlast, __shfl_xor_sync(0xffffffffu, wlast, o));

    for (int c = nchunks - 1; c >= 0; c--) {
        const int base = c * GH_BWD_CHUNK;
        const int cnt = min(GH_BWD_CHUNK, n - base);
        if (c != nchunks - 1) {
            __syncthreads();
#pragma unroll
            for (int h = 0; h < PER_THREAD; h++)
                if (tid + h * GH_BWD_THREADS < GH_BWD_CHUNK) gh_stage_issue_b(st, tid + h * GH_BWD_THREADS, next_id[h], geo, features);
            gh_cp_async_commit();
            if (c > 0) {
#pragma unroll
                for (int h = 0; h < PER_THREAD; h++)
                    if (tid + h * GH_BWD_THREADS < GH_BWD_CHUNK)
                        next_id[h] = (uint32_t)inst[(size_t)rg.x + base - GH_BWD_CHUNK + tid + h * GH_BWD_THREADS];
            }
            gh_cp_async_wait_all();
            __syncthreads();
            for (int word = warp; word * 32 < cnt; word += GH_BWD_THREADS / 32)
                gh_build_lists_b(st, cnt, word, lane, tx0, ty0, base, GH_GLAST_LO, GH_GLAST_HI);
            __syncthreads();
        }
        if ((uint32_t)base >= wlast) continue;

        int wi = (cnt + 31) >> 5;
        uint32_t cur = 0;
        while (true) {
            while (cur == 0 && wi > 0) cur = st.bits[blk][--wi];
            const bool act = (cur != 0);
            if (!__any_sync(0xffffffffu, act)) break;

            const int bpos = act ? 31 - __clz(cur) : 0;
            cur &= ~(1u << bpos);
            const int jj = act ? wi * 32 + bpos : 0;
            const uint32_t id = st.id[jj];
            const float4 g0 = st.g0[jj], g1 = st.g1[jj];
            const float2* feat = &st.feat[jj * GH_HALF_C];
            const uint32_t pos = act ? (uint32_t)(base + jj) : 0xffffffffu;
            float v[16];
            const bool contrib = gh_bwd_pair(pr, g0, g1, feat, pxf, pos, nddelx_dx, nddely_dy, v);
            const uint32_t cm = __ballot_sync(0xffffffffu, contrib);
            if (cm == 0u) continue;
#if GH_BWD_LPB == 4
            const float4 s = gh_group4_reduce16(v, red_buf, lane);
            if ((cm >> gshift) & gmask) {
                float4* dst = reinterpret_cast<float4*>(acc16 + (size_t)id * 16) + (lane & 3);
                atomicAdd(dst, s);
            }
#else
            float4 s0, s1;
            gh_group2_reduce16(v, lane, s0, s1);
            if (GH_ABLATE_REDG ? (s0.x == -1.5e-38f) : ((cm >> gshift) & gmask)) {
#if GH_BWD_RED2_SECTOR
                float4* dst = reinterpret_cast<float4*>(acc16 + (size_t)id * 16) + (lane & 1);
                atomicAdd(dst, s0);
                atomicAdd(dst + 2, s1);
#else
                float4* dst = reinterpret_cast<float4*>(acc16 + (size_t)id * 16) + 2 * (lane & 1);
                atomicAdd(dst, s0);
                atomicAdd(dst + 1, s1);
#endif
            }
#endif
        }
    }
    gh_cp_async_wait_all();
}
#undef GH_GLAST_LO
#undef GH_GLAST_HI

__global__ void __launch_bounds__(256)
gh_unpack_grads_kernel(int P, const float* __restrict__ acc16, float* __restrict__ dL_dmean2D,
                       float* __restrict__ dL_dconic, float* __restrict__ dL_dopacity, float* __restrict__ dL_dcolor,
                       float* __restrict__ dL_dmean3D, float* __restrict__ dL_dcov3D,
                       float* __restrict__ dL_dscale, float* __restrict__ dL_drot)
{
    const int idx = blockIdx.x * blockDim.x + threadIdx.x;
    if (idx >= P) return;
    const float4* a = reinterpret_cast<const float4*>(acc16 + (size_t)idx * 16);
    const float4 a0 = a[0], a1 = a[1], a2 = a[2], a3 = a[3];
    float2* dc = reinterpret_cast<float2*>(dL_dcolor + (size_t)idx * GH_NUM_CHANNELS);
    dc[0] = make_float2(a0.x, a0.y); dc[1] = make_float2(a0.z, a0.w);
    dc[2] = make_float2(a1.x, a1.y); dc[3] = make_float2(a1.z, a1.w);
    dc[4] = make_float2(a2.x, a2.y);
    dL_dmean2D[3 * idx + 0] = a2.z; dL_dmean2D[3 * idx + 1] = a2.w; dL_dmean2D[3 * idx + 2] = 0.f;
    reinterpret_cast<float4*>(dL_dconic)[idx] = make_float4(a3.x, a3.y, 0.f, a3.z);
    dL_dopacity[idx] = a3.w;
    if (dL_dmean3D) { dL_dmean3D[3 * idx + 0] = 0.f; dL_dmean3D[3 * idx + 1] = 0.f; dL_dmean3D[3 * idx + 2] = 0.f; }
    if (dL_dcov3D) {
#pragma unroll
        for (int k = 0; k < 6; k++) dL_dcov3D[6 * idx + k] = 0.f;
    }
    if (dL_dscale) { dL_dscale[3 * idx + 0] = 0.f; dL_dscale[3 * idx + 1] = 0.f; dL_dscale[3 * idx + 2] = 0.f; }
    if (dL_drot) reinterpret_cast<float4*>(dL_drot)[idx] = make_float4(0.f, 0.f, 0.f, 0.f);
}

}

void gh_launch_blend_forward(int W, int H, int gx, int gy, GhGeomWS geom, GhImgWS img, GhBinWS bin,
                             const float* features, const float* bg, float* out_color,
                             cudaStream_t stream)
{
    const int smem = (int)(kFwdSmemBytes > (size_t)GH_FWD_SMEM_MIN ? kFwdSmemBytes : (size_t)GH_FWD_SMEM_MIN);
    cudaFuncSetAttribute(gh_blend_forward_kernel, cudaFuncAttributeMaxDynamicSharedMemorySize, smem);
    cudaFuncSetAttribute(gh_blend_forward_kernel, cudaFuncAttributePreferredSharedMemoryCarveout, 100);
    gh_blend_forward_kernel<<<gx * gy, GH_FWD_THREADS, smem, stream>>>(img.ranges, img.tile_perm, bin.inst, geom.geo, features,
                                                         W, H, gx, bg, img.final_T, img.n_contrib, out_color);
}

void gh_launch_blend_backward(int W, int H, int gx, int gy, GhGeomWS geom, GhImgWS img, GhBinWS bin,
                              const float* features, const float* bg, const float* dL_dpix,
                              cudaStream_t stream)
{
    const int smem = (int)(sizeof(GhStageB) + GH_BWD_THREADS * GH_RED_LANE_STRIDE4 * sizeof(float4));
    cudaFuncSetAttribute(gh_blend_backward_kernel, cudaFuncAttributeMaxDynamicSharedMemorySize, smem);
    cudaFuncSetAttribute(gh_blend_backward_kernel, cudaFuncAttributePreferredSharedMemoryCarveout, 100);
    gh_blend_backward_kernel<<<gx * gy, GH_BWD_THREADS, smem, stream>>>(img.ranges, img.tile_perm, bin.inst, geom.geo, features,
                                                          W, H, gx, bg, img.final_T, img.n_contrib, dL_dpix,
                                                          geom.acc16);
}

void gh_launch_unpack_grads(int P, GhGeomWS geom, float* dL_dmean2D, float* dL_dconic, float* dL_dopacity,
                            float* dL_dcolor, float* dL_dmean3D, float* dL_dcov3D, float* dL_dscale, float* dL_drot,
                            cudaStream_t stream)
{
    gh_unpack_grads_kernel<<<(P + 255) / 256, 256, 0, stream>>>(P, geom.acc16, dL_dmean2D, dL_dconic,
                                                                dL_dopacity, dL_dcolor, dL_dmean3D, dL_dcov3D,
                                                                dL_dscale, dL_drot);
}
```

### gaussianhaircut_b200/csrc/gh_common.cuh

```cuda
#pragma once
#include <cuda_runtime.h>
#include <stdint.h>

#define GH_NUM_CHANNELS 10
#define GH_BLOCK_X 16
#define GH_BLOCK_Y 16
#define GH_TILE_PIX (GH_BLOCK_X * GH_BLOCK_Y)

#define GH_ERR_PREFILTERED 1u

#define GH_MUL(a, b) __fmul_rn((a), (b))
#define GH_ADD(a, b) __fadd_rn((a), (b))
#define GH_SUB(a, b) __fsub_rn((a), (b))
#define GH_FMA(a, b, c) __fmaf_rn((a), (b), (c))
#define GH_DIV(a, b) __fdiv_rn((a), (b))
#define GH_RCP(a) __frcp_rn((a))
#define GH_SQRT(a) __fsqrt_rn((a))

struct __align__(16) GhGeo {
    float x, y, ca, cb;
    float cc, op, thr, pd;
};

struct GhCtrl {
    unsigned int num_rendered;
    unsigned int max_tile_len;
    unsigned int err_flags;
    unsigned int nseg;
};

static __host__ __device__ __forceinline__ size_t gh_align_up(size_t v, size_t a) {
    return (v + a - 1) / a * a;
}

struct GhGeomWS {
    GhGeo* geo;
    float* depth;
    float* acc16;
    static __host__ __device__ size_t bytes(size_t P) {
        return gh_align_up(P * sizeof(GhGeo), 256) + gh_align_up(P * sizeof(float), 256) +
               gh_align_up(P * 64, 256) + 256;
    }
    static __host__ __device__ GhGeomWS carve(char* base, size_t P) {
        GhGeomWS w;
        size_t off = gh_align_up((size_t)base, 256) - (size_t)base;
        w.geo = (GhGeo*)(base + off); off += gh_align_up(P * sizeof(GhGeo), 256);
        w.depth = (float*)(base + off); off += gh_align_up(P * sizeof(float), 256);
        w.acc16 = (float*)(base + off);
        return w;
    }
};

struct GhImgWS {
    GhCtrl* ctrl;
    uint32_t* tile_count;
    uint32_t* tile_cursor;
    uint2* ranges;
    uint32_t* tile_perm;
    float* final_T;
    uint32_t* n_contrib;
    static __host__ __device__ size_t bytes(size_t npix, size_t T) {
        return 256 + 3 * gh_align_up(T * 4, 256) + gh_align_up(T * 8, 256) +
               2 * gh_align_up(npix * 4, 256) + 256;
    }
    static __host__ __device__ GhImgWS carve(char* base, size_t npix, size_t T) {
        GhImgWS w;
        size_t off = gh_align_up((size_t)base, 256) - (size_t)base;
        w.ctrl = (GhCtrl*)(base + off); off += 256;
        w.tile_count = (uint32_t*)(base + off); off += gh_align_up(T * 4, 256);
        w.tile_cursor = (uint32_t*)(base + off); off += gh_align_up(T * 4, 256);
        w.ranges = (uint2*)(base + off); off += gh_align_up(T * 8, 256);
        w.tile_perm = (uint32_t*)(base + off); off += gh_align_up(T * 4, 256);
        w.final_T = (float*)(base + off); off += gh_align_up(npix * 4, 256);
        w.n_contrib = (uint32_t*)(base + off);
        return w;
    }
};

struct GhBinWS {
    uint64_t* inst;
    uint64_t* tmp;
    uint2* seg;
    static __host__ __device__ size_t max_segments(size_t R) { return R / 768 + R / 2048 + 2; }
    static __host__ __device__ size_t bytes(size_t R) {
        return 2 * gh_align_up(R * 8, 256) + gh_align_up(max_segments(R) * 8, 256) + 256;
    }
    static __host__ __device__ GhBinWS carve(char* base, size_t R) {
        GhBinWS w;
        size_t off = gh_align_up((size_t)base, 256) - (size_t)base;
        w.inst = (uint64_t*)(base + off); off += gh_align_up(R * 8, 256);
        w.tmp = (uint64_t*)(base + off); off += gh_align_up(R * 8, 256);
        w.seg = (uint2*)(base + off);
        return w;
    }
};

#ifdef __CUDACC__
__device__ __forceinline__ void gh_get_rect(float px, float py, int radius, int gx, int gy,
                                            int& minx, int& miny, int& maxx, int& maxy) {
    const float rf = (float)radius;
    int v;
    v = __float2int_rz(GH_MUL(GH_SUB(px, rf), 0.0625f)); minx = min(gx, max(0, v));
    v = __float2int_rz(GH_MUL(GH_SUB(py, rf), 0.0625f)); miny = min(gy, max(0, v));
    v = __float2int_rz(GH_MUL(GH_ADD(GH_ADD(GH_ADD(px, rf), 16.0f), -1.0f), 0.0625f)); maxx = min(gx, max(0, v));
    v = __float2int_rz(GH_MUL(GH_ADD(GH_ADD(GH_ADD(py, rf), 16.0f), -1.0f), 0.0625f)); maxy = min(gy, max(0, v));
}

__device__ __forceinline__ float gh_ndc2pix(float v, int S) {
    double t = __dadd_rn((double)v, 1.0);
    t = __fma_rn(t, (double)S, -1.0);
    t = __dmul_rn(t, 0.5);
    return __double2float_rn(t);
}

__device__ __forceinline__ bool gh_pre_project(float px, float py, float pz, const float* __restrict__ vm,
                                               const float* __restrict__ pm, float& zview, float& projx, float& projy) {
    zview = GH_ADD(__ldg(vm + 14), GH_FMA(pz, __ldg(vm + 10), GH_FMA(px, __ldg(vm + 2), GH_MUL(py, __ldg(vm + 6)))));
    if (zview <= 0.2f) return false;
    const float hx = GH_ADD(__ldg(pm + 12), GH_FMA(pz, __ldg(pm + 8), GH_FMA(px, __ldg(pm + 0), GH_MUL(py, __ldg(pm + 4)))));
    const float hy = GH_ADD(__ldg(pm + 13), GH_FMA(pz, __ldg(pm + 9), GH_FMA(px, __ldg(pm + 1), GH_MUL(py, __ldg(pm + 5)))));
    const float hw = GH_ADD(__ldg(pm + 15), GH_FMA(pz, __ldg(pm + 11), GH_FMA(px, __ldg(pm + 3), GH_MUL(py, __ldg(pm + 7)))));
    const float p_w = GH_RCP(GH_ADD(hw, 0.0000001f));
    projx = GH_MUL(hx, p_w); projy = GH_MUL(hy, p_w);
    return true;
}

__device__ __forceinline__ bool gh_pre_from_conic(float conx, float cony, float conz, float& covx, float& covz, float& det) {
    const float det_inv = GH_FMA(conx, conz, -GH_MUL(cony, cony));
    if (det_inv == 0.0f) return false;
    det = GH_RCP(det_inv);
    covx = GH_MUL(conz, det);
    covz = GH_MUL(conx, det);
    return true;
}

__device__ __forceinline__ int gh_pre_finish(float covx, float covz, float det, float conx, float cony, float conz,
                                             float projx, float projy, float op, int W, int H, int gx, int gy,
                                             int& minx, int& miny, int& maxx, int& maxy, GhGeo& g) {
    const float mid = GH_MUL(GH_ADD(covx, covz), 0.5f);
    const float sq = GH_SQRT(fmaxf(GH_FMA(mid, mid, -det), 0.1f));
    const float lam = fmaxf(GH_ADD(mid, sq), GH_SUB(mid, sq));
    const float my_radius = ceilf(GH_MUL(GH_SQRT(lam), 3.0f));
    const float pix_x = gh_ndc2pix(projx, W), pix_y = gh_ndc2pix(projy, H);
    const int ri = __float2int_rz(my_radius);
    if (ri <= 0) return 0;
    int x0, y0, x1, y1;
    gh_get_rect(pix_x, pix_y, ri, gx, gy, x0, y0, x1, y1);
    if ((x1 - x0) * (y1 - y0) == 0) return 0;
    g.x = pix_x; g.y = pix_y; g.ca = conx; g.cb = cony; g.cc = conz; g.op = op;
    g.thr = __logf(255.0f * op);
    g.thr = (255.0f * op > 0.f) ? g.thr : -1e30f;
    const bool pd = (conx > 0.f) && (conz > 0.f) && (conx * conz - cony * cony > 0.f) && (op == op);
    g.pd = pd ? 1.0f : 0.0f;
    if (!(op == op)) g.thr = 1e30f;
    minx = x0; miny = y0; maxx = x1; maxy = y1;
    return ri;
}

__device__ __forceinline__ GhGeo gh_geo_not_rendered() {
    GhGeo g; g.x = 0.f; g.y = 0.f; g.ca = 0.f; g.cb = 0.f; g.cc = 0.f; g.op = 0.f; g.thr = -1e30f; g.pd = 0.f;
    return g;
}

struct GhWarpRects {
    int incl, excl, w, minxy, total;
    uint32_t rw;
};
__device__ __forceinline__ GhWarpRects gh_warp_rects(int minx, int miny, int maxx, int maxy, int lane) {
    GhWarpRects r;
    r.w = maxx - minx;
    const int count = r.w * (maxy - miny);
    int v = count;
#pragma unroll
    for (int o = 1; o < 32; o <<= 1) { const int nb = __shfl_up_sync(0xffffffffu, v, o); if (lane >= o) v += nb; }
    r.incl = v; r.excl = v - count;
    r.total = __shfl_sync(0xffffffffu, v, 31);
    r.minxy = minx | (miny << 16);
    r.rw = (r.w > 1) ? (0xffffffffu / (uint32_t)r.w + 1u) : 0u;
    return r;
}
__device__ __forceinline__ int gh_warp_rect_item(const GhWarpRects& r, int j, int gx, int& owner) {
    int lo = 0;
#pragma unroll
    for (int s = 16; s > 0; s >>= 1) {
        const int v = __shfl_sync(0xffffffffu, r.incl, lo + s - 1);
        if (v <= j) lo += s;
    }
    owner = lo;
    const int oexcl = __shfl_sync(0xffffffffu, r.excl, lo);
    const int ow = __shfl_sync(0xffffffffu, r.w, lo);
    const uint32_t orw = __shfl_sync(0xffffffffu, r.rw, lo);
    const int oxy = __shfl_sync(0xffffffffu, r.minxy, lo);
    const uint32_t k = (uint32_t)(j - oexcl);
    const uint32_t q = (ow > 1) ? __umulhi(k, orw) : k;
    const int x = (oxy & 0xffff) + (int)(k - q * (uint32_t)ow), y = (oxy >> 16) + (int)q;
    return (j < r.total) ? y * gx + x : -1;
}

__device__ __forceinline__ void gh_warp_tile_histogram(int minx, int miny, int maxx, int maxy, int gx,
                                                       uint32_t* __restrict__ tile_count) {
    const int lane = threadIdx.x & 31;
    const GhWarpRects wr = gh_warp_rects(minx, miny, maxx, maxy, lane);
    for (int j0 = 0; j0 < wr.total; j0 += 32) {
        int owner;
        const int tile = gh_warp_rect_item(wr, j0 + lane, gx, owner);
        const uint32_t peers = __match_any_sync(0xffffffffu, tile);
        if (tile >= 0 && lane == __ffs(peers) - 1) atomicAdd(&tile_count[tile], (uint32_t)__popc(peers));
    }
}

__device__ __forceinline__ void gh_cov3d(float s0, float s1, float s2, float mod,
                                         float r, float x, float y, float z, float* cov) {
    const float sx = GH_MUL(mod, s0), sy = GH_MUL(mod, s1), sz = GH_MUL(mod, s2);
    const float yy = GH_MUL(y, y), zz = GH_MUL(z, z);
    const float xz = GH_MUL(x, z), rx = GH_MUL(r, x), rz = GH_MUL(r, z);
    const float yy_zz = GH_ADD(yy, zz);
    const float xx_zz = GH_FMA(x, x, zz);
    const float xx_yy = GH_FMA(x, x, yy);
    const float R00 = GH_SUB(1.0f, GH_ADD(yy_zz, yy_zz));
    const float t01 = GH_FMA(x, y, -rz);   const float R01 = GH_ADD(t01, t01);
    const float t02 = GH_FMA(r, y, xz);    const float R02 = GH_ADD(t02, t02);
    const float t10 = GH_FMA(x, y, rz);    const float R10 = GH_ADD(t10, t10);
    const float R11 = GH_SUB(1.0f, GH_ADD(xx_zz, xx_zz));
    const float t12 = GH_FMA(y, z, -rx);   const float R12 = GH_ADD(t12, t12);
    const float t20 = GH_FMA(-r, y, xz);   const float R20 = GH_ADD(t20, t20);
    const float t21 = GH_FMA(y, z, rx);    const float R21 = GH_ADD(t21, t21);
    const float R22 = GH_SUB(1.0f, GH_ADD(xx_yy, xx_yy));
    const float M00 = GH_MUL(sx, R00), M01 = GH_MUL(sy, R01), M02 = GH_MUL(sz, R02);
    const float M10 = GH_MUL(sx, R10), M11 = GH_MUL(sy, R11), M12 = GH_MUL(sz, R12);
    const float M20 = GH_MUL(sx, R20), M21 = GH_MUL(sy, R21), M22 = GH_MUL(sz, R22);
    cov[0] = GH_FMA(M02, M02, GH_FMA(M00, M00, GH_MUL(M01, M01)));
    cov[1] = GH_FMA(M02, M12, GH_FMA(M00, M10, GH_MUL(M01, M11)));
    cov[2] = GH_FMA(M02, M22, GH_FMA(M00, M20, GH_MUL(M01, M21)));
    cov[3] = GH_FMA(M12, M12, GH_FMA(M10, M10, GH_MUL(M11, M11)));
    cov[4] = GH_FMA(M12, M22, GH_FMA(M10, M20, GH_MUL(M11, M21)));
    cov[5] = GH_FMA(M22, M22, GH_FMA(M20, M20, GH_MUL(M21, M21)));
}

__device__ __forceinline__ float gh_power(float dx, float dy, float ca, float cb, float cc) {
    const float t1 = GH_MUL(dx, ca);
    const float t3 = GH_MUL(dy, GH_MUL(dy, cc));
    const float s = GH_FMA(dx, t1, t3);
    const float t5 = GH_MUL(dy, GH_MUL(dx, cb));
    return GH_FMA(s, -0.5f, -t5);
}

#ifndef GH_INKERNEL_SORT_MAX
#define GH_INKERNEL_SORT_MAX 1792u
#endif
static_assert(GH_INKERNEL_SORT_MAX >= 1675u, "GhBinWS::max_segments assumes long lists of more than 1675 records");
__device__ __forceinline__ void gh_ce(uint64_t& a, uint64_t& b) {
    const uint64_t lo = a < b ? a : b, hi = a < b ? b : a;
    a = lo; b = hi;
}

template <typename KeyPtr>
__device__ __forceinline__ void gh_bitonic_sort(KeyPtr keys, const uint32_t n, const int tid, const int nt)
{
    const uint64_t INF = ~0ull;
    uint32_t ln2 = 0;
    while ((1u << ln2) < n) ln2++;
    const uint32_t half = (1u << ln2) >> 1, quarter = half >> 1;
    for (uint32_t lk = 1; lk <= ln2; lk++) {
        {
            const uint32_t k = 1u << lk, hk = k >> 1;
            for (uint32_t t = tid; t < half; t += nt) {
                const uint32_t blk = t >> (lk - 1), off = t & (hk - 1);
                const uint32_t i = (blk << lk) + off, j = (blk << lk) + (k - 1 - off);
                if (j < n) {
                    const uint64_t a = keys[i], b = keys[j];
                    if (a > b) { keys[i] = b; keys[j] = a; }
                }
            }
            __syncthreads();
        }
        int ls = (int)lk - 2;
        for (; ls >= 1; ls -= 2) {
            const uint32_t sft = (uint32_t)ls, s = 1u << sft, h = s >> 1;
            for (uint32_t t = tid; t < quarter; t += nt) {
                const uint32_t i = ((t >> (sft - 1)) << (sft + 1)) | (t & (h - 1));
                if (i < n) {
                    const uint32_t ib = i + h, ic = i + s, id = ic + h;
                    uint64_t ka = keys[i];
                    uint64_t kb = ib < n ? keys[ib] : INF;
                    uint64_t kc = ic < n ? keys[ic] : INF;
                    uint64_t kd = id < n ? keys[id] : INF;
                    gh_ce(ka, kc); gh_ce(kb, kd);
                    gh_ce(ka, kb); gh_ce(kc, kd);
                    keys[i] = ka;
                    if (ib < n) keys[ib] = kb;
                    if (ic < n) keys[ic] = kc;
                    if (id < n) keys[id] = kd;
                }
            }
            __syncthreads();
        }
        if (ls == 0) {
            for (uint32_t t = tid; t < half; t += nt) {
                const uint32_t i = t << 1, j = i + 1;
                if (j < n) {
                    const uint64_t a = keys[i], b = keys[j];
                    if (a > b) { keys[i] = b; keys[j] = a; }
                }
            }
            __syncthreads();
        }
    }
}

#define GH_SORT_SUB 1024u
#define GH_SORT_SCRATCH_WORDS (GH_SORT_SUB + 512u)
template <int NT>
__device__ __forceinline__ void gh_bucket_sort_tile(uint64_t* A, uint64_t* B, uint32_t* cnt, int n, int tid) {
    constexpr int NW = NT / 32;
    constexpr int V4 = (int)GH_SORT_SUB / 4 / NT;
    __shared__ uint32_t s_red[16];
    __shared__ uint32_t s_nbig;
    const int lane = tid & 31, warp = tid >> 5;
    uint32_t* big = cnt + GH_SORT_SUB;
    uint32_t dmin = 0xffffffffu, dmax = 0u;
    for (int i = tid; i < n; i += NT) { const uint32_t d = (uint32_t)(A[i] >> 32); dmin = min(dmin, d); dmax = max(dmax, d); }
#pragma unroll
    for (int o = 16; o > 0; o >>= 1) {
        dmin = min(dmin, __shfl_xor_sync(0xffffffffu, dmin, o));
        dmax = max(dmax, __shfl_xor_sync(0xffffffffu, dmax, o));
    }
    if (lane == 0) { s_red[warp] = dmin; s_red[8 + warp] = dmax; }
#pragma unroll
    for (int q = 0; q < V4; q++) reinterpret_cast<uint4*>(cnt)[tid * V4 + q] = make_uint4(0u, 0u, 0u, 0u);
    if (tid == 0) s_nbig = 0u;
    __syncthreads();
#pragma unroll
    for (int w = 0; w < NW; w++) { dmin = min(dmin, s_red[w]); dmax = max(dmax, s_red[8 + w]); }
    const float inv = (float)GH_SORT_SUB / ((float)(dmax - dmin) + 1.0f);
    for (int i = tid; i < n; i += NT) {
        const uint32_t d = (uint32_t)(A[i] >> 32);
        const uint32_t b = min(GH_SORT_SUB - 1u, (uint32_t)((float)(d - dmin) * inv));
        atomicAdd(&cnt[b], 1u);
    }
    __syncthreads();
    int r0, r1;
    {
        uint4 c[V4];
        uint32_t sum = 0;
#pragma unroll
        for (int q = 0; q < V4; q++) { c[q] = reinterpret_cast<uint4*>(cnt)[tid * V4 + q]; sum += c[q].x + c[q].y + c[q].z + c[q].w; }
        uint32_t v = sum;
#pragma unroll
        for (int o = 1; o < 32; o <<= 1) { const uint32_t nb = __shfl_up_sync(0xffffffffu, v, o); if (lane >= o) v += nb; }
        if (lane == 31) s_red[warp] = v;
        __syncthreads();
        uint32_t start = v - sum;
#pragma unroll
        for (int w = 0; w < NW; w++) start += (w < warp) ? s_red[w] : 0u;
        r0 = (int)start; r1 = (int)(start + sum);
        uint32_t run = start;
#pragma unroll
        for (int q = 0; q < V4; q++) {
            const uint4 cur = make_uint4(run, run + c[q].x, run + c[q].x + c[q].y, run + c[q].x + c[q].y + c[q].z);
            run += c[q].x + c[q].y + c[q].z + c[q].w;
            reinterpret_cast<uint4*>(cnt)[tid * V4 + q] = cur;
        }
    }
    __syncthreads();
    for (int i = tid; i < n; i += NT) {
        const uint64_t key = A[i];
        const uint32_t d = (uint32_t)(key >> 32);
        const uint32_t b = min(GH_SORT_SUB - 1u, (uint32_t)((float)(d - dmin) * inv));
        B[atomicAdd(&cnt[b], 1u)] = key;
    }
    __syncthreads();
    if (r1 - r0 > 32) {
        const uint32_t q = atomicAdd(&s_nbig, 1u);
        big[2 * q] = (uint32_t)r0; big[2 * q + 1] = (uint32_t)(r1 - r0);
    } else {
        for (int i = r0 + 1; i < r1; i++) {
            const uint64_t key = B[i];
            int j = i - 1;
            while (j >= r0 && B[j] > key) { B[j + 1] = B[j]; j--; }
            B[j + 1] = key;
        }
    }
    __syncthreads();
    const uint32_t nbig = s_nbig;
    for (uint32_t q = 0; q < nbig; q++)
        gh_bitonic_sort(B + big[2 * q], big[2 * q + 1], tid, NT);
    for (int i = tid; i < n; i += NT) A[i] = B[i];
    __syncthreads();
}

#endif
```

### include/gh_rasterizer.h

```cpp
#ifndef GH_RASTERIZER_H_INCLUDED
#define GH_RASTERIZER_H_INCLUDED

#include <stddef.h>

#ifdef __cplusplus
extern "C" {
#endif

#define GH_NUM_CHANNELS_ABI 10

#define GH_OK 0
#define GH_E_INVALID_ARG 1
#define GH_E_NO_COLORS 2
#define GH_E_CUDA 3
#define GH_E_PREFILTERED 4

typedef void* gh_stream_t;

int gh_abi_version(void);

int gh_num_channels(void);

unsigned long long gh_kernel_launch_count(void);

void gh_stage_timing_enable(int on);
int gh_stage_timing_read(double* ms_sum, unsigned long long* calls, int capacity);

const char* gh_last_error(void);

int gh_forward_workspace_sizes(int P, int width, int height, size_t* geom_bytes, size_t* img_bytes);

int gh_binning_workspace_size(long long R, size_t* binning_bytes);

int gh_forward_preprocess(
    int P, int D, int M,
    int width, int height,
    const float* means3D, const float* means2D_precomp, const float* shs,
    const float* colors_precomp, const float* opacities,
    const float* scales, float scale_modifier, const float* rotations,
    const float* cov3D_precomp, const float* conic_precomp,
    const float* viewmatrix, const float* projmatrix, const float* cam_pos,
    float tan_fovx, float tan_fovy, int prefiltered,
    int* radii,
    char* geom_buffer, char* img_buffer,
    int* num_rendered, int* max_tile_len,
    int debug, gh_stream_t stream);

int gh_forward_render(
    int P, int width, int height,
    const float* background, const float* colors_precomp,
    const int* radii,
    char* geom_buffer, char* binning_buffer, char* img_buffer,
    int num_rendered, int max_tile_len,
    float* out_color,
    int debug, gh_stream_t stream);

int gh_backward(
    int P, int D, int M, int R,
    int width, int height,
    const float* background,
    const float* means3D, const float* shs, const float* colors_precomp,
    const float* scales, float scale_modifier, const float* rotations,
    const float* cov3D_precomp, const float* conic_precomp,
    const float* viewmatrix, const float* projmatrix, const float* campos,
    float tan_fovx, float tan_fovy,
    const int* radii,
    char* geom_buffer, char* binning_buffer, char* img_buffer,
    const float* dL_dpix,
    float* dL_dmean2D, float* dL_dconic, float* dL_dopacity, float* dL_dcolor,
    float* dL_dmean3D, float* dL_dcov3D, float* dL_dsh, float* dL_dscale, float* dL_drot,
    int debug, gh_stream_t stream);

int gh_mark_visible(int P, const float* means3D, const float* viewmatrix, const float* projmatrix,
                    unsigned char* present, gh_stream_t stream);

int gh_debug_export(
    int P, int width, int height, long long R,
    const char* geom_buffer, const char* binning_buffer, const char* img_buffer,
    unsigned long long* keys_sorted, unsigned int* point_list, unsigned int* ranges,
    float* final_T, unsigned int* n_contrib,
    float* depths, float* means2D, float* conic_opacity,
    gh_stream_t stream);

#define GH_ADAM_MAX_GROUPS 8
int gh_adam_step(int n_groups, float* const* params, const float* const* grads,
                 float* const* exp_avg, float* const* exp_avg_sq,
                 const unsigned long long* sizes, const float* lrs,
                 float beta1, float beta2, float eps, int step, int* step_state,
                 unsigned int* nan_flag, const unsigned int* skip_flag, gh_stream_t stream);

int gh_image_loss_workspace_size(int width, int height, size_t* bytes);
int gh_image_loss(int width, int height, const float* out_color, const float* gt_image,
                  const float* gt_mask, const float* gt_orient_angle, const float* gt_orient_conf,
                  float lambda_dl1, float lambda_dssim, float lambda_dmask, float lambda_dorient,
                  void* workspace, float* losses, float* dL_dout, gh_stream_t stream);

int gh_allreduce_p2p(const unsigned long long* peer_bufs, const unsigned long long* peer_flags,
                     unsigned long long multicast_buf, int rank, int world,
                     size_t offset_floats, size_t n_floats, unsigned int epoch,
                     unsigned int* local_sync, unsigned int* nan_out, gh_stream_t stream);

int gh_project_workspace_size(int P, size_t* bytes);
int gh_project_forward(
    int P, int width, int height,
    const float* xyz, const float* scaling, const float* rotation, const float* dirs,
    const float* features_dc, const float* features_rest,
    const float* opacity, const float* label, const float* orient_conf,
    const float* viewmatrix, const float* projmatrix, const float* campos,
    float tan_fovx, float tan_fovy, float scale_modifier, int sh_degree, unsigned int flags, float det_eps,
    float* means2D, float* colors, float* opacities, float* conic, float* cov3D, unsigned char* visible,
    gh_stream_t stream);
int gh_project_forward_binned(
    int P, int width, int height,
    const float* xyz, const float* scaling, const float* rotation, const float* dirs,
    const float* features_dc, const float* features_rest,
    const float* opacity, const float* label, const float* orient_conf,
    const float* viewmatrix, const float* projmatrix, const float* campos,
    float tan_fovx, float tan_fovy, float scale_modifier, int sh_degree, unsigned int flags, float det_eps,
    float* means2D, float* colors, float* opacities, float* conic, float* cov3D, unsigned char* visible,
    int* radii, char* geom_buffer, char* img_buffer, int* num_rendered, int* max_tile_len,
    gh_stream_t stream);
int gh_project_backward(
    int P, int width, int height,
    const float* xyz, const float* scaling, const float* rotation, const float* dirs,
    const float* features_dc, const float* features_rest,
    const float* opacity, const float* label, const float* orient_conf,
    const float* viewmatrix, const float* projmatrix, const float* campos,
    float tan_fovx, float tan_fovy, float scale_modifier, int sh_degree, unsigned int flags, float det_eps,
    const unsigned char* visible,
    const char* geom_buffer,
    const float* dL_dmeans2D, const float* dL_dconic, const float* dL_dcolors, const float* dL_dopacity,
    float* d_xyz, float* d_scaling, float* d_rotation, float* d_dirs, float* d_features_dc, float* d_features_rest,
    float* d_opacity, float* d_label, float* d_orient_conf, float* d_means2D, float* d_camera,
    unsigned int* nan_flag, void* workspace, gh_stream_t stream);

int gh_densify_classify(int P, const float* grad_accum, const float* denom, const float* log_scaling,
                        const float* opacity_logit, float grad_threshold, float dense_extent,
                        float min_opacity, float ws_limit, int* flags, gh_stream_t stream);
int gh_densify_scatter(int P, int n_tensors, const float* const* src, const float* const* exp_avg,
                       const float* const* exp_avg_sq, float* const* dst, float* const* dst_exp_avg,
                       float* const* dst_exp_avg_sq, const int* row_floats,
                       int xyz_index, int scaling_index, int rotation_index,
                       const int* flags, const int* inclusive_prefix, int n_keep, int n_clone, int n_split_kept,
                       const float* samples, int n_split_all, gh_stream_t stream);

#ifdef __cplusplus
}
#endif
#endif
```

Before: 827.2 million.

## Record per-pair 2x2 block masks and tile last index in forward for backward reuse

The forward blend kernel now records, for every (tile, Gaussian) pair, a 64-bit mask of which 2x2 pixel blocks actually blended it, plus the tile's last contributing index. It writes these into the binning tmp buffer and the tile_cursor slot. The backward kernel reads these masks instead of recomputing conservative per-block ellipse masks and per-pixel n_contrib maxima, so it does less ALU work and skips pairs that never contributed. The cost is extra global writes and a deferred flush in the forward pass. It also reuses scratch buffers that must no longer be live, and it drops the configurable LPB=4 path.

Result: no change. 830.5 million, median of 6 (+0.4%).

```diff
diff --git a/gaussianhaircut_b200/_C.py b/gaussianhaircut_b200/_C.py
--- a/gaussianhaircut_b200/_C.py
+++ b/gaussianhaircut_b200/_C.py
@@ -287,3 +287,15 @@
             _ptr(out["final_T"]), _ptr(out["n_contrib"]),
             _ptr(out["depths"]), _ptr(out["means2D"]), _ptr(out["conic_opacity"]), _stream(device)))
     return out
+
+
+def debug_export_blend_masks(W: int, H: int, R: int, binningBuffer, imgBuffer):
+    lib = _capi.load()
+    device = imgBuffer.device
+    T = ((W + 15) // 16) * ((H + 15) // 16)
+    tile_last = torch.zeros(T, dtype=torch.int32, device=device)
+    block_mask = torch.zeros(R, dtype=torch.int64, device=device)
+    with torch.cuda.device(device):
+        _capi.check(lib.gh_debug_export_blend_masks(W, H, R, _ptr(binningBuffer), _ptr(imgBuffer),
+                                                    _ptr(tile_last), _ptr(block_mask), _stream(device)))
+    return tile_last, block_mask
diff --git a/gaussianhaircut_b200/_capi.py b/gaussianhaircut_b200/_capi.py
--- a/gaussianhaircut_b200/_capi.py
+++ b/gaussianhaircut_b200/_capi.py
@@ -97,6 +97,7 @@
     "gh_densify_classify": (_i, [_i, _p, _p, _p, _p, _f, _f, _f, _f, _p, _p]),
     "gh_densify_scatter": (_i, [_i, _i, _p, _p, _p, _p, _p, _p, _p, _i, _i, _i, _p, _p, _i, _i, _i, _p, _i, _p]),
     "gh_debug_export": (_i, [_i, _i, _i, _ll, _p, _p, _p, _p, _p, _p, _p, _p, _p, _p, _p, _p]),
+    "gh_debug_export_blend_masks": (_i, [_i, _i, _ll, _p, _p, _p, _p, _p]),
 }
 
 _lib = None
diff --git a/gaussianhaircut_b200/csrc/gh_api.cu b/gaussianhaircut_b200/csrc/gh_api.cu
--- a/gaussianhaircut_b200/csrc/gh_api.cu
+++ b/gaussianhaircut_b200/csrc/gh_api.cu
@@ -356,4 +356,24 @@
     return GH_OK;
 }
 
-}
+int gh_debug_export_blend_masks(int width, int height, long long R, const char* binning_buffer, const char* img_buffer,
+                                unsigned int* tile_last, unsigned int* block_mask, gh_stream_t stream_)
+{
+    cudaStream_t stream = (cudaStream_t)stream_;
+    g_err[0] = 0;
+    if (width <= 0 || height <= 0 || R < 0 || !img_buffer || (R > 0 && block_mask && !binning_buffer))
+        return gh_fail(GH_E_INVALID_ARG, "gh_debug_export_blend_masks: bad arguments");
+    int gx, gy; gh_grid(width, height, gx, gy);
+    const int T = gx * gy;
+    GhImgWS img = GhImgWS::carve(const_cast<char*>(img_buffer), (size_t)width * height, (size_t)T);
+    cudaError_t e = cudaSuccess;
+    if (tile_last) e = cudaMemcpyAsync(tile_last, img.tile_last, (size_t)T * 4, cudaMemcpyDeviceToDevice, stream);
+    if (R > 0 && block_mask && e == cudaSuccess) {
+        GhBinWS bin = GhBinWS::carve(const_cast<char*>(binning_buffer), (size_t)R);
+        e = cudaMemcpyAsync(block_mask, bin.blk, (size_t)R * 8, cudaMemcpyDeviceToDevice, stream);
+    }
+    if (e != cudaSuccess) return gh_check_cuda(e, "debug export (blend masks)");
+    return GH_OK;
+}
+
+}
diff --git a/gaussianhaircut_b200/csrc/gh_blend.cu b/gaussianhaircut_b200/csrc/gh_blend.cu
--- a/gaussianhaircut_b200/csrc/gh_blend.cu
+++ b/gaussianhaircut_b200/csrc/gh_blend.cu
@@ -24,13 +24,8 @@
 #ifndef GH_BWD_MIN_CTAS
 #define GH_BWD_MIN_CTAS 6
 #endif
-#ifndef GH_BWD_LPB
-#define GH_BWD_LPB 2
-#endif
-#define GH_BWD_NBLK (128 / GH_BWD_LPB)
-#define GH_BWD_BPW (32 / GH_BWD_LPB)
-#define GH_BWD_BW GH_BWD_LPB
-#define GH_BWD_NBX (16 / GH_BWD_BW)
+#define GH_BWD_NBLK 64
+#define GH_BWD_BPW 16
 #ifndef GH_ABLATE_REDG
 #define GH_ABLATE_REDG 0
 #endif
@@ -182,11 +177,12 @@
                         const GhGeo* __restrict__ geo, const float* __restrict__ features,
                         int W, int H, int gx, const float* __restrict__ bg,
                         float* __restrict__ final_T, uint32_t* __restrict__ n_contrib,
-                        float* __restrict__ out)
+                        float* __restrict__ out, uint2* __restrict__ blk_out, uint32_t* __restrict__ tile_last)
 {
     extern __shared__ __align__(16) unsigned char gh_fwd_smem[];
     GhStage& st = *reinterpret_cast<GhStage*>(gh_fwd_smem);
     uint32_t* pairbits = reinterpret_cast<uint32_t*>(gh_fwd_smem + sizeof(GhStage));
+    __shared__ uint32_t s_wlast[GH_FWD_THREADS / 32];
 
     const int tile = GH_TILE_ORDER ? (int)tile_perm[blockIdx.x] : (int)blockIdx.x;
     const int tx = tile % gx, ty = tile / gx;
@@ -283,8 +279,22 @@
 #if GH_FWD_NBUF == 2
     if (nchunks > 0) stage_window(0, 0);
 #endif
-
-    for (int c = 0; c < nchunks; c++) {
+    auto flush_window = [&](int cw) {
+        const int wbase = cw * GH_FWD_CHUNK, wcnt = min(GH_FWD_CHUNK, n - wbase);
+        for (int word = warp; word * 32 < wcnt; word += GH_FWD_THREADS / 32) {
+            uint32_t m[2];
+#pragma unroll
+            for (int half = 0; half < 2; half++) {
+                const uint32_t* pw = pairbits + word * GH_FWD_THREADS + (2 * half + (lane >> 4)) * 32 + 2 * (lane & 15);
+                const uint32_t x = pw[0] | pw[1];
+                m[half] = __any_sync(0xffffffffu, x != 0u) ? gh_transpose32(x, lane) : 0u;
+            }
+            if (word * 32 + lane < wcnt) blk_out[(size_t)rg.x + wbase + word * 32 + lane] = make_uint2(m[0], m[1]);
+        }
+    };
+
+    int c = 0;
+    for (; c < nchunks; c++) {
         const int base = c * GH_FWD_CHUNK;
         const int cnt = min(GH_FWD_CHUNK, n - base);
         const int nwords = (cnt + 31) >> 5;
@@ -293,10 +303,12 @@
         gh_cp_async_wait_all();
         if (__syncthreads_and(warp_done)) break;
         if (c + 1 < nchunks) stage_window(c + 1, buf ^ 1);
+        if (c > 0) flush_window(c - 1);
 #else
         constexpr int buf = 0;
         if (__syncthreads_and(warp_done)) break;
         stage_window(c, 0);
+        if (c > 0) flush_window(c - 1);
         gh_cp_async_wait_all();
         __syncthreads();
 #endif
@@ -305,19 +317,20 @@
                 gh_build_pair_lists(st, pairbits, buf, cnt, word, lane, tx0, ty0);
         __syncthreads();
 
+        uint32_t nz = 0u;
+#pragma unroll
+        for (int k = 0; k < GH_FWD_WORDS; k++)
+            if (k < nwords) nz |= (pairbits[k * GH_FWD_THREADS + tid] != 0u) ? (1u << k) : 0u;
         if (!(done0 && done1) && !GH_ABLATE_TRAVERSE) {
-            uint32_t nz = 0u;
-#pragma unroll
-            for (int k = 0; k < GH_FWD_WORDS; k++)
-                if (k < nwords) nz |= (pairbits[k * GH_FWD_THREADS + tid] != 0u) ? (1u << k) : 0u;
             int wi = 0;
-            uint32_t cur = 0u;
+            uint32_t cur = 0u, blended = 0u;
             while (true) {
                 if (cur == 0u) {
                     if (nz == 0u) break;
                     wi = __ffs(nz) - 1;
                     nz &= nz - 1;
                     cur = pairbits[wi * GH_FWD_THREADS + tid];
+                    blended = 0u;
                 }
                 const int bpos = __ffs(cur) - 1;
                 cur &= cur - 1;
@@ -347,13 +360,25 @@
                     T = make_float2(blend0 ? test_T.x : T.x, blend1 ? test_T.y : T.y);
                     last0 = blend0 ? pos : last0;
                     last1 = blend1 ? pos : last1;
+                    blended |= 1u << bpos;
                 }
+                if (cur == 0u || (done0 && done1)) pairbits[wi * GH_FWD_THREADS + tid] = blended;
                 if (done0 && done1) break;
             }
         }
+        for (; nz != 0u; nz &= nz - 1) pairbits[(__ffs(nz) - 1) * GH_FWD_THREADS + tid] = 0u;
         warp_done = (__ballot_sync(0xffffffffu, done0 && done1) == 0xffffffffu);
     }
     gh_cp_async_wait_all();
+    __syncthreads();
+    if (c > 0) flush_window(c - 1);
+
+    uint32_t wl = max(last0, last1);
+#pragma unroll
+    for (int o = 16; o > 0; o >>= 1) wl = max(wl, __shfl_xor_sync(0xffffffffu, wl, o));
+    if (lane == 0) s_wlast[warp] = wl;
+    __syncthreads();
+    if (tid == 0) tile_last[tile] = max(max(s_wlast[0], s_wlast[1]), max(s_wlast[2], s_wlast[3]));
 
     const size_t plane = (size_t)H * W;
 #pragma unroll
@@ -388,125 +413,19 @@
     st.id[slot] = id;
 }
 
-#if GH_BWD_LPB == 4
-__device__ __forceinline__ uint32_t gh_block_mask2(const float4 g0, const float4 g1, float tx0, float ty0) {
-    const float gx = g0.x, gy = g0.y, a = g0.z, b = g0.w, c = g1.x, thr = g1.z, pd = g1.w;
-    if (pd == 0.f) return 0xffffffffu;
-    const float mxd = fmaxf(fabsf(gx - tx0), fabsf(gx - (tx0 + 15.f)));
-    const float myd = fmaxf(fabsf(gy - ty0), fabsf(gy - (ty0 + 15.f)));
-    const float slack = 1e-3f + 2e-5f * (a * mxd * mxd + c * myd * myd + 2.f * fabsf(b) * mxd * myd);
-    const float Q = 2.f * (thr + slack);
-    if (!(Q >= 0.f)) return (Q != Q) ? 0xffffffffu : 0u;
-    const float2 ia = gh_f2(__frcp_rn(a)), aQ = gh_f2(a * Q), bbac = gh_f2(b * b - a * c), gx2 = gh_f2(gx), b2 = gh_f2(b);
-    float2 dy = make_float2(gy - ty0, gy - (ty0 + 1.f));
-    uint32_t mask = 0;
-#pragma unroll
-    for (int by = 0; by < 8; by++) {
-        const float2 disc = gh_fma2(gh_mul2(dy, dy), bbac, aQ);
-        const float2 s = gh_mul2(disc, make_float2(rsqrtf(disc.x), rsqrtf(disc.y)));
-        const float2 hb = gh_mul2(b2, dy);
-        const float2 lo2 = gh_fma2(gh_sub2(hb, s), ia, gx2), hi2 = gh_fma2(gh_add2(hb, s), ia, gx2);
-        const float xlo = fminf(fminf(1e30f, lo2.x), lo2.y), xhi = fmaxf(fmaxf(-1e30f, hi2.x), hi2.y);
-        const float lo = (xlo - 0.01f) - tx0, hi = (xhi + 0.01f) - tx0;
-        const int p0 = max(0, __float2int_ru(lo)), p1 = min(15, __float2int_rd(hi));
-        if (p0 <= p1) {
-            const int b0 = p0 >> 2, b1 = p1 >> 2;
-            mask |= (((2u << (b1 - b0)) - 1u) << b0) << (4 * by);
-        }
-        dy = gh_add2(dy, gh_f2(-2.f));
-    }
-    return mask;
-}
-#endif
-
-#if GH_BWD_LPB != 4
-__device__ __forceinline__ uint2 gh_block_mask_2x2(const float4 g0, const float4 g1, float tx0, float ty0) {
-    const float gx = g0.x, gy = g0.y, a = g0.z, b = g0.w, c = g1.x, thr = g1.z, pd = g1.w;
-    if (pd == 0.f) return make_uint2(0xffffffffu, 0xffffffffu);
-    const float mxd = fmaxf(fabsf(gx - tx0), fabsf(gx - (tx0 + 15.f)));
-    const float myd = fmaxf(fabsf(gy - ty0), fabsf(gy - (ty0 + 15.f)));
-    const float slack = 1e-3f + 2e-5f * (a * mxd * mxd + c * myd * myd + 2.f * fabsf(b) * mxd * myd);
-    const float Q = 2.f * (thr + slack);
-    if (!(Q >= 0.f)) return (Q != Q) ? make_uint2(0xffffffffu, 0xffffffffu) : make_uint2(0u, 0u);
-    const float2 ia = gh_f2(__frcp_rn(a)), aQ = gh_f2(a * Q), bbac = gh_f2(b * b - a * c), gx2 = gh_f2(gx), b2 = gh_f2(b);
-    float2 dy = make_float2(gy - ty0, gy - (ty0 + 1.f));
-    uint32_t m[2] = {0u, 0u};
-#pragma unroll 1
-    for (int half = 0; half < 2; half++) {
-        uint32_t mh = 0u;
-#pragma unroll
-        for (int by = 0; by < 4; by++) {
-            const float2 disc = gh_fma2(gh_mul2(dy, dy), bbac, aQ);
-            const float2 s = gh_mul2(disc, make_float2(rsqrtf(disc.x), rsqrtf(disc.y)));
-            const float2 hb = gh_mul2(b2, dy);
-            const float2 lo2 = gh_fma2(gh_sub2(hb, s), ia, gx2), hi2 = gh_fma2(gh_add2(hb, s), ia, gx2);
-            const float xlo = fminf(fminf(1e30f, lo2.x), lo2.y), xhi = fmaxf(fmaxf(-1e30f, hi2.x), hi2.y);
-            const float lo = (xlo - 0.01f) - tx0, hi = (xhi + 0.01f) - tx0;
-            const int p0 = max(0, __float2int_ru(lo)), p1 = min(15, __float2int_rd(hi));
-            if (p0 <= p1) {
-                const int b0 = p0 >> 1, b1 = p1 >> 1;
-                mh |= (((2u << (b1 - b0)) - 1u) << b0) << (8 * by);
-            }
-            dy = gh_add2(dy, gh_f2(-2.f));
-        }
-        if (half == 0) m[0] = mh; else m[1] = mh;
-    }
-    return make_uint2(m[0], m[1]);
-}
-#endif
-
-__device__ __forceinline__ uint32_t gh_valid_bits(uint32_t glast, int first_pos) {
-    const int lim = (int)glast - first_pos;
-    return lim >= 32 ? 0xffffffffu : (lim <= 0 ? 0u : ((1u << lim) - 1u));
-}
-
-__device__ __forceinline__ void gh_build_lists_b(GhStageB& st, int cnt, int word, int lane, float tx0, float ty0,
-                                                 int base, uint32_t glast_lo, uint32_t glast_hi) {
-    const int j = word * 32 + lane;
-#if GH_BWD_LPB == 4
-    uint32_t m = 0;
-    if (j < cnt) m = gh_block_mask2(st.g0[j], st.g1[j], tx0, ty0);
-    uint32_t mine = 0;
-    if (__any_sync(0xffffffffu, m != 0u)) mine = gh_transpose32(m, lane);
-    st.bits[lane][word] = mine & gh_valid_bits(glast_lo, base + word * 32);
-    (void)glast_hi;
-#else
-    uint2 m = make_uint2(0u, 0u);
-    if (j < cnt) m = gh_block_mask_2x2(st.g0[j], st.g1[j], tx0, ty0);
+__device__ __forceinline__ void gh_build_lists_b(GhStageB& st, uint2 m, int word, int lane) {
     uint32_t lo = 0, hi = 0;
     if (__any_sync(0xffffffffu, m.x != 0u)) lo = gh_transpose32(m.x, lane);
     if (__any_sync(0xffffffffu, m.y != 0u)) hi = gh_transpose32(m.y, lane);
-    st.bits[lane][word] = lo & gh_valid_bits(glast_lo, base + word * 32);
-    st.bits[32 + lane][word] = hi & gh_valid_bits(glast_hi, base + word * 32);
-#endif
+    st.bits[lane][word] = lo;
+    st.bits[32 + lane][word] = hi;
 }
 
 #define GH_BWD_THREADS 128
-
-#define GH_RED_STRIDE4 5
-#if GH_BWD_LPB == 4
-__device__ __forceinline__ float4 gh_group4_reduce16(const float (&v)[16], float4* warp_buf, int lane) {
-    float4* mine = warp_buf + lane * GH_RED_STRIDE4;
-    mine[0] = make_float4(v[0], v[1], v[2], v[3]);
-    mine[1] = make_float4(v[4], v[5], v[6], v[7]);
-    mine[2] = make_float4(v[8], v[9], v[10], v[11]);
-    mine[3] = make_float4(v[12], v[13], v[14], v[15]);
-    __syncwarp();
-    const float4* grp = warp_buf + (lane & 28) * GH_RED_STRIDE4 + (lane & 3);
-    const float4 a = grp[0], b = grp[GH_RED_STRIDE4], c = grp[2 * GH_RED_STRIDE4], d = grp[3 * GH_RED_STRIDE4];
-    __syncwarp();
-    const float2 lo = gh_add2(gh_add2(make_float2(a.x, a.y), make_float2(b.x, b.y)),
-                              gh_add2(make_float2(c.x, c.y), make_float2(d.x, d.y)));
-    const float2 hi = gh_add2(gh_add2(make_float2(a.z, a.w), make_float2(b.z, b.w)),
-                              gh_add2(make_float2(c.z, c.w), make_float2(d.z, d.w)));
-    return make_float4(lo.x, lo.y, hi.x, hi.y);
-}
-#endif
 
 #ifndef GH_BWD_RED2_SECTOR
 #define GH_BWD_RED2_SECTOR 1
 #endif
-#if GH_BWD_LPB != 4
 __device__ __forceinline__ void gh_group2_reduce16(const float (&v)[16], int lane, float4& out0, float4& out1) {
     const bool odd = (lane & 1) != 0;
     constexpr int H = GH_BWD_RED2_SECTOR ? 4 : 8;
@@ -520,12 +439,6 @@
     out0 = make_float4(k[0], k[1], k[2], k[3]);
     out1 = make_float4(k[4], k[5], k[6], k[7]);
 }
-#endif
-#if GH_BWD_LPB == 4
-#define GH_RED_LANE_STRIDE4 GH_RED_STRIDE4
-#else
-#define GH_RED_LANE_STRIDE4 0
-#endif
 
 struct GhBwdPair {
     float2 T, A, last_alpha, last_cdot;
@@ -591,7 +504,9 @@
 }
 
 __global__ void __launch_bounds__(GH_BWD_THREADS, GH_BWD_MIN_CTAS)
-gh_blend_backward_kernel(const uint2* __restrict__ ranges, const uint32_t* __restrict__ tile_perm, const uint64_t* __restrict__ inst,
+gh_blend_backward_kernel(const uint2* __restrict__ ranges, const uint32_t* __restrict__ tile_perm,
+                         const uint32_t* __restrict__ tile_last, const uint64_t* __restrict__ inst,
+                         const uint2* __restrict__ blk_in,
                          const GhGeo* __restrict__ geo, const float* __restrict__ features,
                          int W, int H, int gx, const float* __restrict__ bg,
                          const float* __restrict__ final_T, const uint32_t* __restrict__ n_contrib,
@@ -600,70 +515,48 @@
 {
     extern __shared__ __align__(16) unsigned char gh_bwd_smem[];
     GhStageB& st = *reinterpret_cast<GhStageB*>(gh_bwd_smem);
-#if GH_BWD_LPB == 4
-    float4* red_buf = reinterpret_cast<float4*>(gh_bwd_smem + sizeof(GhStageB)) + (threadIdx.x >> 5) * 32 * GH_RED_LANE_STRIDE4;
-#endif
-    __shared__ uint32_t s_warp_last[GH_BWD_THREADS / 32];
-    __shared__ uint32_t s_glast[GH_BWD_NBLK];
     __shared__ uint8_t s_perm[GH_BWD_THREADS / 32][GH_BWD_NBLK];
 
     const int tile = GH_TILE_ORDER ? (int)tile_perm[blockIdx.x] : (int)blockIdx.x;
     const int tx = tile % gx, ty = tile / gx;
     const int tid = threadIdx.x, lane = tid & 31, warp = tid >> 5;
-    const float tx0 = (float)(tx * GH_BLOCK_X), ty0 = (float)(ty * GH_BLOCK_Y);
-    const unsigned gshift = lane & (32 - GH_BWD_LPB);
-    const unsigned gmask = (1u << GH_BWD_LPB) - 1u;
+    const unsigned gshift = lane & 30;
     const size_t plane = (size_t)H * W;
-    const uint2 rg = ranges[tile];
-
-    {
-        const int nb = GH_BWD_BPW * warp + lane / GH_BWD_LPB;
-        const int nx = tx * GH_BLOCK_X + GH_BWD_BW * (nb % GH_BWD_NBX) + (lane % GH_BWD_LPB);
-        const int ny = ty * GH_BLOCK_Y + 2 * (nb / GH_BWD_NBX);
-        uint32_t gl = 0;
-        if (nx < W && ny < H) gl = n_contrib[(size_t)ny * W + nx];
-        if (nx < W && ny + 1 < H) gl = max(gl, n_contrib[(size_t)(ny + 1) * W + nx]);
-#pragma unroll
-        for (int o = GH_BWD_LPB / 2; o > 0; o >>= 1) gl = max(gl, __shfl_xor_sync(0xffffffffu, gl, o));
-        if ((lane % GH_BWD_LPB) == 0) s_glast[nb] = gl;
-        uint32_t wl = gl;
-#pragma unroll
-        for (int o = GH_BWD_LPB; o < 32; o <<= 1) wl = max(wl, __shfl_xor_sync(0xffffffffu, wl, o));
-        if (lane == 0) s_warp_last[warp] = wl;
-    }
-    __syncthreads();
-    uint32_t tile_last = 0;
-#pragma unroll
-    for (int w = 0; w < GH_BWD_THREADS / 32; w++) tile_last = max(tile_last, s_warp_last[w]);
-    const int n = (int)tile_last;
+    const int n = (int)tile_last[tile];
+    if (n == 0) return;
+    const size_t list0 = ranges[tile].x;
     const int nchunks = (n + GH_BWD_CHUNK - 1) / GH_BWD_CHUNK;
-    if (nchunks == 0) return;
     constexpr int PER_THREAD = (GH_BWD_CHUNK + GH_BWD_THREADS - 1) / GH_BWD_THREADS;
-#define GH_GLAST_LO s_glast[lane]
-#define GH_GLAST_HI ((GH_BWD_NBLK > 32) ? s_glast[(32 + lane) % GH_BWD_NBLK] : 0u)
 
     uint32_t next_id[PER_THREAD];
-    {
-        const int base = (nchunks - 1) * GH_BWD_CHUNK;
-        const int cnt = n - base;
+    uint2 next_m[PER_THREAD];
+    auto fetch_window = [&](int c) {
+        const int base = c * GH_BWD_CHUNK, cnt = min(GH_BWD_CHUNK, n - base);
 #pragma unroll
         for (int h = 0; h < PER_THREAD; h++) {
             const int slot = tid + h * GH_BWD_THREADS;
-            if (slot < cnt) gh_stage_issue_b(st, slot, (uint32_t)inst[(size_t)rg.x + base + slot], geo, features);
+            const bool in = slot < cnt;
+            next_id[h] = in ? (uint32_t)inst[list0 + base + slot] : 0u;
+            next_m[h] = in ? blk_in[list0 + base + slot] : make_uint2(0u, 0u);
+        }
+    };
+    auto stage_window = [&](int c) {
+        const int cnt = min(GH_BWD_CHUNK, n - c * GH_BWD_CHUNK);
+#pragma unroll
+        for (int h = 0; h < PER_THREAD; h++) {
+            const int slot = tid + h * GH_BWD_THREADS;
+            if (slot == 0 || (next_m[h].x | next_m[h].y) != 0u) gh_stage_issue_b(st, slot, next_id[h], geo, features);
         }
         gh_cp_async_commit();
-        if (nchunks > 1) {
-#pragma unroll
-            for (int h = 0; h < PER_THREAD; h++)
-                if (tid + h * GH_BWD_THREADS < GH_BWD_CHUNK)
-                    next_id[h] = (uint32_t)inst[(size_t)rg.x + base - GH_BWD_CHUNK + tid + h * GH_BWD_THREADS];
-        }
+#pragma unroll
+        for (int h = 0; h < PER_THREAD; h++)
+            if ((warp + 4 * h) * 32 < cnt) gh_build_lists_b(st, next_m[h], warp + 4 * h, lane);
+        if (c > 0) fetch_window(c - 1);
         gh_cp_async_wait_all();
         __syncthreads();
-        for (int word = warp; word * 32 < cnt; word += GH_BWD_THREADS / 32)
-            gh_build_lists_b(st, cnt, word, lane, tx0, ty0, base, GH_GLAST_LO, GH_GLAST_HI);
-        __syncthreads();
-    }
+    };
+    fetch_window(nchunks - 1);
+    stage_window(nchunks - 1);
 
     int blk;
     {
@@ -671,27 +564,24 @@
         uint32_t len0 = 0, len1 = 0;
         for (int w = 0; w < nw; w++) {
             len0 += __popc(st.bits[lane][w]);
-            if (GH_BWD_NBLK > 32) len1 += __popc(st.bits[(32 + lane) % GH_BWD_NBLK][w]);
+            len1 += __popc(st.bits[32 + lane][w]);
         }
         const uint32_t key0 = (len0 << 6) | (uint32_t)lane, key1 = (len1 << 6) | (uint32_t)(32 + lane);
         int rank0 = 0, rank1 = 0;
 #pragma unroll
         for (int k = 0; k < 32; k++) {
             const uint32_t a = __shfl_sync(0xffffffffu, key0, k);
-            rank0 += (a < key0) ? 1 : 0;
-            if (GH_BWD_NBLK > 32) {
-                const uint32_t b = __shfl_sync(0xffffffffu, key1, k);
-                rank0 += (b < key0) ? 1 : 0;
-                rank1 += ((a < key1) ? 1 : 0) + ((b < key1) ? 1 : 0);
-            }
+            const uint32_t b = __shfl_sync(0xffffffffu, key1, k);
+            rank0 += ((a < key0) ? 1 : 0) + ((b < key0) ? 1 : 0);
+            rank1 += ((a < key1) ? 1 : 0) + ((b < key1) ? 1 : 0);
         }
         s_perm[warp][rank0] = (uint8_t)lane;
-        if (GH_BWD_NBLK > 32) s_perm[warp][rank1] = (uint8_t)(32 + lane);
+        s_perm[warp][rank1] = (uint8_t)(32 + lane);
         __syncwarp();
-        blk = s_perm[warp][GH_BWD_BPW * warp + lane / GH_BWD_LPB];
-    }
-    const int px = tx * GH_BLOCK_X + GH_BWD_BW * (blk % GH_BWD_NBX) + (lane % GH_BWD_LPB);
-    const int py0 = ty * GH_BLOCK_Y + 2 * (blk / GH_BWD_NBX);
+        blk = s_perm[warp][GH_BWD_BPW * warp + lane / 2];
+    }
+    const int px = tx * GH_BLOCK_X + 2 * (blk % 8) + (lane & 1);
+    const int py0 = ty * GH_BLOCK_Y + 2 * (blk / 8);
     const float pxf = (float)px;
 
     GhBwdPair pr;
@@ -726,32 +616,13 @@
     }
     const float nddelx_dx = -0.5f * W, nddely_dy = -0.5f * H;
 
-    uint32_t wlast = s_glast[blk];
-#pragma unroll
-    for (int o = GH_BWD_LPB; o < 32; o <<= 1) wlast = max(wlast, __shfl_xor_sync(0xffffffffu, wlast, o));
-
     for (int c = nchunks - 1; c >= 0; c--) {
         const int base = c * GH_BWD_CHUNK;
         const int cnt = min(GH_BWD_CHUNK, n - base);
         if (c != nchunks - 1) {
             __syncthreads();
-#pragma unroll
-            for (int h = 0; h < PER_THREAD; h++)
-                if (tid + h * GH_BWD_THREADS < GH_BWD_CHUNK) gh_stage_issue_b(st, tid + h * GH_BWD_THREADS, next_id[h], geo, features);
-            gh_cp_async_commit();
-            if (c > 0) {
-#pragma unroll
-                for (int h = 0; h < PER_THREAD; h++)
-                    if (tid + h * GH_BWD_THREADS < GH_BWD_CHUNK)
-                        next_id[h] = (uint32_t)inst[(size_t)rg.x + base - GH_BWD_CHUNK + tid + h * GH_BWD_THREADS];
-            }
-            gh_cp_async_wait_all();
-            __syncthreads();
-            for (int word = warp; word * 32 < cnt; word += GH_BWD_THREADS / 32)
-                gh_build_lists_b(st, cnt, word, lane, tx0, ty0, base, GH_GLAST_LO, GH_GLAST_HI);
-            __syncthreads();
-        }
-        if ((uint32_t)base >= wlast) continue;
+            stage_window(c);
+        }
 
         int wi = (cnt + 31) >> 5;
         uint32_t cur = 0;
@@ -771,16 +642,9 @@
             const bool contrib = gh_bwd_pair(pr, g0, g1, feat, pxf, pos, nddelx_dx, nddely_dy, v);
             const uint32_t cm = __ballot_sync(0xffffffffu, contrib);
             if (cm == 0u) continue;
-#if GH_BWD_LPB == 4
-            const float4 s = gh_group4_reduce16(v, red_buf, lane);
-            if ((cm >> gshift) & gmask) {
-                float4* dst = reinterpret_cast<float4*>(acc16 + (size_t)id * 16) + (lane & 3);
-                atomicAdd(dst, s);
-            }
-#else
             float4 s0, s1;
             gh_group2_reduce16(v, lane, s0, s1);
-            if (GH_ABLATE_REDG ? (s0.x == -1.5e-38f) : ((cm >> gshift) & gmask)) {
+            if (GH_ABLATE_REDG ? (s0.x == -1.5e-38f) : ((cm >> gshift) & 3u)) {
 #if GH_BWD_RED2_SECTOR
                 float4* dst = reinterpret_cast<float4*>(acc16 + (size_t)id * 16) + (lane & 1);
                 atomicAdd(dst, s0);
@@ -791,13 +655,10 @@
                 atomicAdd(dst + 1, s1);
 #endif
             }
-#endif
         }
     }
     gh_cp_async_wait_all();
 }
-#undef GH_GLAST_LO
-#undef GH_GLAST_HI
 
 __global__ void __launch_bounds__(256)
 gh_unpack_grads_kernel(int P, const float* __restrict__ acc16, float* __restrict__ dL_dmean2D,
@@ -835,17 +696,19 @@
     cudaFuncSetAttribute(gh_blend_forward_kernel, cudaFuncAttributeMaxDynamicSharedMemorySize, smem);
     cudaFuncSetAttribute(gh_blend_forward_kernel, cudaFuncAttributePreferredSharedMemoryCarveout, 100);
     gh_blend_forward_kernel<<<gx * gy, GH_FWD_THREADS, smem, stream>>>(img.ranges, img.tile_perm, bin.inst, geom.geo, features,
-                                                         W, H, gx, bg, img.final_T, img.n_contrib, out_color);
+                                                         W, H, gx, bg, img.final_T, img.n_contrib, out_color,
+                                                         bin.blk, img.tile_last);
 }
 
 void gh_launch_blend_backward(int W, int H, int gx, int gy, GhGeomWS geom, GhImgWS img, GhBinWS bin,
                               const float* features, const float* bg, const float* dL_dpix,
                               cudaStream_t stream)
 {
-    const int smem = (int)(sizeof(GhStageB) + GH_BWD_THREADS * GH_RED_LANE_STRIDE4 * sizeof(float4));
+    const int smem = (int)sizeof(GhStageB);
     cudaFuncSetAttribute(gh_blend_backward_kernel, cudaFuncAttributeMaxDynamicSharedMemorySize, smem);
     cudaFuncSetAttribute(gh_blend_backward_kernel, cudaFuncAttributePreferredSharedMemoryCarveout, 100);
-    gh_blend_backward_kernel<<<gx * gy, GH_BWD_THREADS, smem, stream>>>(img.ranges, img.tile_perm, bin.inst, geom.geo, features,
+    gh_blend_backward_kernel<<<gx * gy, GH_BWD_THREADS, smem, stream>>>(img.ranges, img.tile_perm, img.tile_last, bin.inst,
+                                                          bin.blk, geom.geo, features,
                                                           W, H, gx, bg, img.final_T, img.n_contrib, dL_dpix,
                                                           geom.acc16);
 }
diff --git a/gaussianhaircut_b200/csrc/gh_common.cuh b/gaussianhaircut_b200/csrc/gh_common.cuh
--- a/gaussianhaircut_b200/csrc/gh_common.cuh
+++ b/gaussianhaircut_b200/csrc/gh_common.cuh
@@ -55,6 +55,7 @@
     GhCtrl* ctrl;
     uint32_t* tile_count;
     uint32_t* tile_cursor;
+    uint32_t* tile_last;
     uint2* ranges;
     uint32_t* tile_perm;
     float* final_T;
@@ -69,6 +70,7 @@
         w.ctrl = (GhCtrl*)(base + off); off += 256;
         w.tile_count = (uint32_t*)(base + off); off += gh_align_up(T * 4, 256);
         w.tile_cursor = (uint32_t*)(base + off); off += gh_align_up(T * 4, 256);
+        w.tile_last = w.tile_cursor;
         w.ranges = (uint2*)(base + off); off += gh_align_up(T * 8, 256);
         w.tile_perm = (uint32_t*)(base + off); off += gh_align_up(T * 4, 256);
         w.final_T = (float*)(base + off); off += gh_align_up(npix * 4, 256);
@@ -80,6 +82,7 @@
 struct GhBinWS {
     uint64_t* inst;
     uint64_t* tmp;
+    uint2* blk;
     uint2* seg;
     static __host__ __device__ size_t max_segments(size_t R) { return R / 768 + R / 2048 + 2; }
     static __host__ __device__ size_t bytes(size_t R) {
@@ -90,6 +93,7 @@
         size_t off = gh_align_up((size_t)base, 256) - (size_t)base;
         w.inst = (uint64_t*)(base + off); off += gh_align_up(R * 8, 256);
         w.tmp = (uint64_t*)(base + off); off += gh_align_up(R * 8, 256);
+        w.blk = (uint2*)w.tmp;
         w.seg = (uint2*)(base + off);
         return w;
     }
diff --git a/include/gh_rasterizer.h b/include/gh_rasterizer.h
--- a/include/gh_rasterizer.h
+++ b/include/gh_rasterizer.h
@@ -82,6 +82,10 @@
     float* depths, float* means2D, float* conic_opacity,
     gh_stream_t stream);
 
+int gh_debug_export_blend_masks(
+    int width, int height, long long R, const char* binning_buffer, const char* img_buffer,
+    unsigned int* tile_last, unsigned int* block_mask, gh_stream_t stream);
+
 #define GH_ADAM_MAX_GROUPS 8
 int gh_adam_step(int n_groups, float* const* params, const float* const* grads,
                  float* const* exp_avg, float* const* exp_avg_sq,
```
